# coralogix/arrow-ballista

Hardware: AMD Instinct MI355X
Metric: tpch_sf100_q3_lineitem_rows_per_sec (higher is better)
Workload: dtype i128; 1 GPU; TPC-H SF100 q3 (BASELINE configs[2]): filter x3 + hash join customer|x|orders + hash join |x| lineitem + aggregate + sort, one task on 1 x MI355X; lineitem_rows=600037902, lineitem_rows_per_gpu=600037902, orders_rows_per_gpu=150009476, customer_rows_per_gpu=15000000, input=Arrow-physical columns resident in HBM, parallelism=single partition

## Files before the change

### arrow-ballista_amd/csrc/agg_compile.cpp

```cpp
#include "agg_compile.h"
#include <algorithm>
#include <cctype>
#include <cstdio>
#include <functional>

namespace gpuq {

gpuq_field_info make_field(const std::string& name, const DType& t, bool nullable) {
  gpuq_field_info f{};
  std::snprintf(f.name, sizeof(f.name), "%s", name.c_str());
  f.type = t.id; f.precision = t.p; f.scale = t.s; f.nullable = nullable;
  f.repr = (t.id == T_UTF8) ? GPUQ_REPR_PACKED15 : GPUQ_REPR_ARROW;
  f.width = (t.id == T_BOOL) ? 0 : type_width(t);
  return f;
}

KeySpec make_keyspec(const std::vector<int>& regs, const std::vector<DType>& types, bool null_word) {
  if (regs.size() > (size_t)MAX_KEYS) throw Unsupported("more than " + std::to_string(MAX_KEYS) + " key columns");
  KeySpec K{};
  K.n_keys = (int)regs.size(); K.null_word = null_word ? 1 : 0;
  int w = 0;
  for (size_t k = 0; k < regs.size(); ++k) {
    K.key_reg[k] = regs[k];
    const bool wide = types[k].id == T_DECIMAL128 || types[k].id == T_UTF8;
// ... 395 lines not shown

}

AggCompiled compile_aggregate(const Schema& in, const Json& d) {
  AggCompiled R;
  R.mode = d.get_str("mode", "Single");
  const bool is_final = (R.mode == "Final" || R.mode == "FinalPartitioned");
  const bool emit_state = (R.mode == "Partial");
  if (!is_final && !emit_state && R.mode != "Single") throw std::runtime_error("unknown aggregate mode '" + R.mode + "'");
  R.strategy = d.get_str("strategy", "auto");
  R.expected_groups = d.get_i64("expected_groups", 0);
  Scan s(in);
  ExprCompiler& ec = s.ec;
  if (d.has("predicate")) ec.add_predicate(ec.from_json(d.at("predicate")));
  std::vector<NodeP> declared; std::vector<std::string> declared_names;
  if (d.has("group_expr")) for (const Json& g : d.at("group_expr").a) {
    declared.push_back(ec.from_json(g.at("expr"))); declared_names.push_back(g.get_str("name", "group" + std::to_string(declared.size() - 1)));
  }
  const GroupKeys keys(ec, declared, declared_names);
  R.refuse = keys.refuse;
  s.ungrouped = keys.nodes.empty();
  States states{ec, keys.declared(), in.fields.size()};
  std::vector<AggPlan> plans;
  for (const Json& a : d.at("aggr_expr").a) {
    s.fn = a.at("fn").str(); s.desc = &a;
    AggPlan pl; pl.name = a.get_str("name", s.fn);
    for (auto& ch : s.fn) ch = (char)std::toupper(ch);
    if (a.get_bool("distinct", false)) throw Unsupported("DISTINCT aggregates are not supported on device");
    pl.fn = find_agg_fn(s.fn);
    if (!is_final) {
      NodeP arg = a.has("expr") ? ec.from_json(a.at("expr")) : nullptr;
      if (a.has("filter") && !a.at("filter").is_null()) {
        NodeP p = ec.from_json(a.at("filter"));
        if (p->type.id != T_BOOL) throw std::runtime_error("aggregate FILTER must be boolean");
        if (!arg) arg = ec.lit_int(I64, 1);
        arg = ec.select(p, arg, ec.lit_null(arg->type));
        if (a.has("expr2")) throw Unsupported("FILTER on a two-argument aggregate");
      }
      if (!arg && !(pl.fn && pl.fn->args == 0)) throw std::runtime_error(s.fn + " needs an argument");
      if (!pl.fn) throw Unsupported("aggregate function " + s.fn);
      pl.fn->parts.from_args(s, pl, arg);
    } else {
      if (!pl.fn) throw Unsupported("aggregate function " + s.fn);
      pl.fn->parts.from_states(s, pl, states);
    }
    plans.push_back(pl);
  }
  std::vector<AccDef>& accs = s.accs;
  if (accs.empty()) s.count(nullptr);
  std::vector<int> key_slots, acc_slots(accs.size(), -1);
  for (auto& k : keys.nodes) key_slots.push_back(ec.add_output(k));
  for (size_t i = 0; i < accs.size(); ++i) if (accs[i].arg) acc_slots[i] = ec.add_output(accs[i].arg);
  R.prog = ec.finish();
  if (!s.origin_of.empty()) {
    if (d.has("predicate")) s.pick.add_predicate(ec.from_json(d.at("predicate")));
    R.pick = s.pick.finish();
    R.n_origins = (int)s.origin_of.size();
  }
  const int nk = (int)keys.nodes.size();
  R.agg.n_keys = nk; R.agg.n_accs = (int)accs.size();
  std::vector<int> kregs; bool any_null_key = false;
  for (int k = 0; k < nk; ++k) {
    const NodeP& n = keys.nodes[k];
    R.agg.key_reg[k] = R.prog.out_reg[key_slots[k]]; kregs.push_back(R.agg.key_reg[k]);
    R.key_types.push_back(n->type); any_null_key = any_null_key || n->nullable;
    if (n->type.id == T_BOOL || n->type.id == T_NULL) throw Unsupported("group-by key of type " + n->type.to_string());
  }
  for (size_t i = 0; i < accs.size(); ++i) {
    R.agg.acc_kind[i] = accs[i].kind; R.agg.acc_reg[i] = accs[i].arg ? R.prog.out_reg[acc_slots[i]] : 0;
    R.acc_types.push_back(accs[i].type);
    R.acc_bits.push_back(accs[i].arg ? R.prog.out_bits[acc_slots[i]] : 1);
  }
  R.keys = make_keyspec(kregs, R.key_types, any_null_key);
  {
    int total = 0; bool narrow = nk > 0;
    for (int k = 0; k < nk && narrow; ++k) {
      int bits = 0; bool sgn = false;
      switch (keys.nodes[k]->type.id) {
        case T_INT8: bits = 8; sgn = true; break;   case T_UINT8: bits = 8; break;
        case T_INT16: bits = 16; sgn = true; break; case T_UINT16: bits = 16; break;
        case T_INT32: case T_DATE32: bits = 32; sgn = true; break; case T_UINT32: bits = 32; break;
        default: narrow = false;
      }
      R.keys.sk_bits[k] = bits; R.keys.sk_signed[k] = sgn; R.keys.sk_null[k] = keys.nodes[k]->nullable ? 1 : 0;
      total += bits + R.keys.sk_null[k];
    }
    R.keys.state_key = narrow && total <= 62;
  }

  for (int k = 0; k < nk; ++k) { Field f; f.name = keys.names[k]; f.type = keys.nodes[k]->type; f.nullable = keys.nodes[k]->nullable; f.raw128 = 1; R.post_schema.fields.push_back(f); }
  for (size_t i = 0; i < accs.size(); ++i) { Field f; f.name = "acc" + std::to_string(i); f.type = accs[i].type; f.nullable = false; f.raw128 = 1; R.post_schema.fields.push_back(f); }
  std::function<void(size_t, size_t, bool)> emit = [&](size_t lo, size_t hi, bool with_keys) {
    ExprCompiler pc(R.post_schema);
    std::vector<std::string> names; CompiledProgram cp;
    try {
      if (with_keys) keys.project(pc, names);
      Post p{pc, nk, accs, names};
      for (size_t pi = lo; pi < hi; ++pi) (emit_state ? plans[pi].fn->parts.states : plans[pi].fn->parts.value)(p, plans[pi]);
      cp = pc.finish();
    }
    catch (const Unsupported&) { throw; }
    catch (const std::runtime_error&) {
      if (hi - lo + (with_keys ? 1 : 0) <= 1) throw;
      if (with_keys && hi > lo) { emit(lo, lo, true); emit(lo, hi, false); }
      else { const size_t mid = lo + (hi - lo) / 2; emit(lo, mid, with_keys); emit(mid, hi, false); }
      return;
// ... 12 lines not shown
```

### arrow-ballista_amd/csrc/agg_compile.h

```cpp
#pragma once
#include "../../include/gpuq.h"
#include "expr_compile.h"
#include "gpuq_kernels.h"
#include <string>
#include <vector>

namespace gpuq {

gpuq_field_info make_field(const std::string& name, const DType& t, bool nullable);
KeySpec make_keyspec(const std::vector<int>& regs, const std::vector<DType>& types, bool null_word);

struct AggCompiled {
  std::string mode = "Single", strategy = "auto";
  i64 expected_groups = 0;
  CompiledProgram prog;
  CompiledProgram pick; int n_origins = 0;
  AggSpec agg{}; KeySpec keys{};
  std::vector<DType> key_types, acc_types;
  std::vector<int> acc_bits;
  Schema post_schema;
  struct Post { CompiledProgram prog; int first_out = 0; };
  std::vector<Post> posts;
  std::vector<gpuq_field_info> out_fields;
  std::string refuse;
};
AggCompiled compile_aggregate(const Schema& in, const Json& descriptor);

}
```

### arrow-ballista_amd/csrc/capi.cpp

```cpp
#include "../../include/gpuq.h"
#include "expr_compile.h"
#include "agg_compile.h"
#include "gpuq_kernels.h"
#include "jit_runtime.h"
#include "devbuf.h"
#include "gpuq_internal.h"
#include <hip/hip_runtime.h>
#include <algorithm>
#include <memory>
#include <mutex>
#include <cctype>
#include <cstddef>
#include <cstdio>
#include <cstdlib>
#include <cstring>
#include <string>
#include <tuple>
#include <map>
#include <deque>
#include <functional>
#include <vector>

using namespace gpuq;

namespace {

thread_local std::string g_last_error;

u64 next_pow2(u64 v) { u64 r = 1; while (r < v) r <<= 1; return r; }

}


struct gpuq_timer { hipEvent_t a = nullptr, b = nullptr; };

enum OpKind { K_FILTER, K_PROJECT, K_AGG, K_JOIN_BUILD, K_JOIN_PROBE, K_SORT, K_PARTITION };

struct PassBufs {
  DevBuf hist, look; size_t look_bytes = 0;
  static size_t guess_word_at() { return (size_t)sort_max_passes() * 256; }
  u64* counts(bool with_guess_word = false) { return (u64*)hist.ensure((guess_word_at() + (with_guess_word ? 1 : 0)) * 8); }
  const u64* guess_word() const { return hist.as<u64>() + guess_word_at(); }
  void* lookback(i64 n) { look_bytes = onesweep_ws_bytes(n); return look.ensure(look_bytes); }
};

struct gpuq_op {
  gpuq_ctx* ctx = nullptr;
  OpKind kind = K_FILTER;
  Schema in_schema;
  CompiledProgram prog;
  DevBuf code_dev, flags_dev;
  std::vector<gpuq_field_info> out_fields;
  std::string mode = "Single", strategy = "auto";
  AggSpec agg{}; KeySpec keys{};
  std::vector<DType> key_types, acc_types;
  std::vector<int> acc_bits;
  std::map<std::pair<const void*, int>, int> jit_runs;
  std::map<std::tuple<const void*, int, size_t>, const JitFn*> jit_fns;
  struct PostChunk { CompiledProgram prog; DevBuf code; int first_out = 0; };
  std::deque<PostChunk> posts; Schema post_schema;
  CompiledProgram pick; DevBuf pick_code, origins_dev, origin_rows; int n_origins = 0;
  i64 expected_groups = 0;
  int agg_path = 0;
  int join_type = JT_INNER; int null_eq = 0; bool build_side_rows = true;
  bool has_semi = false; KeySpec semi_keys{};
  SortSpec sort{}; i64 fetch = -1;
  uint32_t nparts = 0;
  struct { void* data = nullptr; u64* valid = nullptr; bool done = false; } sort_dec;
  DType sort_key0;
  std::string refuse;
  std::string label;
  bool deferred = false, defer_client = false;
  struct Learned {
    struct { bool valid = false, dense = false, sparse_bits = false, has_dups = false; i64 kmin = 0; u64 krange = 0; } jb;
    struct { bool valid = false; int path = 0, gmax = 0; u64 est = 0; bool use_lds = false; i64 groups = -1; } ag;
    struct { bool valid = false; SortPack K{}; int total = 0; } so;
    bool join_guess_failed = false, sort_guess_failed = false;
    bool agg_runs_failed = false;
    uint32_t expect_flags = 0;
    void forget() { jb.valid = ag.valid = so.valid = false; }
  } learned;
  struct { DevBuf bitmap, counts, total; } w_filter;
  struct { DevBuf keys, key_nulls, cells, tiny, table, soa, sample, fstage, runs; } w_agg;
  struct { DevBuf key_range; } w_build;
  struct { DevBuf seg_build, seg_probe, counts, rec, rec2, hist, scan, locality; } w_probe;
  struct { DevBuf blocks, klo, klo2, khi, ids, ids2; PassBufs pass; DevBuf khi2, pairs; } w_sort;
  struct { DevBuf pid, pid2; PassBufs pass; DevBuf counts; } w_part;
  uint32_t* pin = nullptr;
  uint32_t* pinned() { if (!pin) { if (hipHostMalloc((void**)&pin, 256, hipHostMallocDefault) != hipSuccess) { (void)hipGetLastError(); pin = nullptr; } } return pin; }
  bool profile = false; hipEvent_t ev0 = nullptr, ev1 = nullptr; float kernel_ms = 0; int launches = 0; bool ev_pending = false;
  hipEvent_t ev2 = nullptr, ev3 = nullptr; float total_ms = 0, last_total_ms = 0; bool ev_total_pending = false;
  ~gpuq_op() { for (hipEvent_t e : {ev0, ev1, ev2, ev3}) if (e) (void)hipEventDestroy(e); if (pin) (void)hipHostFree(pin); }
};

struct gpuq_join_table {
  gpuq_ctx* ctx = nullptr;
  KeySpec keys{}; HashTable T{}; int null_eq = 0; bool has_present = true;
  DevBuf slots, dense, dense_bits, next, visited, present, ws_bitmap, ws_counts;
  i64 bound = 0;
  bool visited_ready = false;
  bool has_dups = false;
};

namespace {

template <class F> int guarded(gpuq_ctx*, F&& f) { return guarded_into(g_last_error, f); }

thread_local bool g_upload = true;
void upload_code(const CompiledProgram& p, DevBuf& dst) {
  if (!g_upload) return;
  dst.ensure(sizeof(DevCode));
  HIPCHECK(hipMemcpy(dst.p, &p.code, sizeof(DevCode), hipMemcpyHostToDevice));
}

DevProgram bind_program(const CompiledProgram& cp, const Schema& schema, const DevCode* code_dev, uint32_t* flags_dev, const gpuq_input* in) {
  if (!in) throw std::runtime_error("input is NULL");
  if (in->n_cols != (int)schema.fields.size())
    throw std::runtime_error("input has " + std::to_string(in->n_cols) + " columns, operator expects " + std::to_string(schema.fields.size()));
  if (in->n_via < 0 || in->n_via > MAX_VIA) throw std::runtime_error("n_via out of range");
  if (in->n_rows < 0 || in->n_rows > 0xFFFFFFFEll) throw std::runtime_error("n_rows out of range (max 2^32-2 positions per call)");
  DevProgram P{};
  P.n_cols = (int)cp.col_field.size(); P.n_insns = cp.n_insns; P.pred_reg = cp.pred_reg; P.n_via = in->n_via;
  for (int k = 0; k < in->n_via; ++k) { if (!in->via[k] && in->n_rows > 0) throw std::runtime_error("index vector is NULL"); P.via[k] = in->via[k]; }
  P.code = code_dev; P.flags = flags_dev; P.n_dev = (const u64*)in->n_rows_dev;
  for (size_t c = 0; c < cp.col_field.size(); ++c) {
    const int fi = cp.col_field[c];
    const Field& f = schema.fields[fi];
    const gpuq_column& col = in->cols[fi];
    if (col.type != f.type.id || (f.type.id == T_DECIMAL128 && (col.precision != f.type.p || col.scale != f.type.s)))
      throw std::runtime_error("column '" + f.name + "': type does not match the operator's input schema (" + f.type.to_string() + ")");
    if (f.side > in->n_via) throw std::runtime_error("column '" + f.name + "' needs index vector " + std::to_string(f.side));
    if (!col.data && col.length > 0 && in->n_rows > 0) throw std::runtime_error("column '" + f.name + "': data is NULL");
    if (!f.nullable && f.side == 0 && col.validity) {  }
    DevCol& d = P.cols[c];
    d.data = col.data; d.offsets = col.offsets; d.validity = col.validity;
    d.cls = f.raw128 ? CC_I128 : col_class_for(f.type);
    if (d.cls == CC_STR && !f.raw128 && !col.offsets && col.length > 0) throw std::runtime_error("Utf8 column '" + f.name + "' has no offsets");
    if (f.raw128 && f.type.id == T_UTF8) d.cls = CC_I128;
    if (d.cls == CC_STR && c < cp.col_loose.size() && cp.col_loose[c]) d.cls = CC_STRQ;
    d.via = f.side;
  }
  return P;
}

DevProgram bind_input(gpuq_op* op, const gpuq_input* in) { return bind_program(op->prog, op->in_schema, op->code_dev.as<DevCode>(), op->flags_dev.as<uint32_t>(), in); }
void check_payload_via(int payload_via, const gpuq_input* in) { if (payload_via < 0 || payload_via > in->n_via) throw std::runtime_error("payload_via out of range"); }
void check_row_limit(i64 n, const char* what) { if (n >= (1ll << 31)) throw Unsupported(std::string(what) + " of >= 2^31 rows in one call"); }
void need_exact_rows(const gpuq_input* in, const char* what) {
  if (in && in->n_rows_dev) throw std::runtime_error(std::string(what) + ": the input carries a device-side row count (n_rows_dev); this entry point needs the exact count");
}
struct OpStatus { uint32_t flags = 0, pad0 = 0, n_groups = 0, pad1 = 0; };
uint32_t* n_groups_dev(gpuq_op* op) { return op->flags_dev.as<uint32_t>() + offsetof(OpStatus, n_groups) / 4; }
void reset_flags(gpuq_op* op, hipStream_t s) { HIPCHECK(hipMemsetAsync(op->flags_dev.p, 0, 4, s)); }
OpStatus read_status(gpuq_op* op, hipStream_t s, int words = 4) {
  OpStatus st; uint32_t* h = op->pinned();
  HIPCHECK(hipMemcpyAsync(h ? (void*)h : (void*)&st, op->flags_dev.p, (size_t)words * 4, hipMemcpyDeviceToHost, s));
  HIPCHECK(hipStreamSynchronize(s));
  if (h) std::memcpy(&st, h, (size_t)words * 4);
  return st;
}
uint32_t read_flags(gpuq_op* op, hipStream_t s) { return read_status(op, s, 1).flags; }
void raise_flags(uint32_t f) {
  if (f & FLAG_STR_TRUNC) throw LongString("a Utf8 value longer than 15 bytes reached a device string comparison/key (PACKED15 limit)");
  if (f & FLAG_DEC_OVERFLOW) throw std::runtime_error("decimal arithmetic overflow: a result or a rescaled operand does not fit Decimal128 (38 digits / 127 bits)");
  if (f & FLAG_WIDE_MINMAX) throw Unsupported("MIN/MAX over a value outside the int64 range is not supported on device");
  if (f & FLAG_DUP_BUILD_KEY) throw Unsupported("duplicate build keys without a chain buffer");
  if (f & FLAG_OUT_OVERFLOW) throw Capacity("join output capacity exceeded; see the pair count for the required size");
  if (f & FLAG_TABLE_FULL) throw std::runtime_error("hash table full");
  if (f & FLAG_GROUP_OVERFLOW) throw Capacity("group capacity exceeded");
  if (f & FLAG_SORT_LAYOUT) throw std::runtime_error("a row does not fit the remembered sort key layout");
  if (f & FLAG_AGG_RUNS) throw std::runtime_error("the aggregate's input is not clustered on its key");
}
uint32_t raise_unless(gpuq_op* op, hipStream_t s, uint32_t f, uint32_t tolerated = 0) {
  if (f & ~tolerated) { reset_flags(op, s); raise_flags(f & ~tolerated); }
  return f & tolerated;
}

struct ProfScope {
  gpuq_op* op; hipStream_t s;
  ProfScope(gpuq_op* o, hipStream_t st) : op(o), s(st) {
    if (op->profile) {
      if (!op->ev0) { HIPCHECK(hipEventCreate(&op->ev0)); HIPCHECK(hipEventCreate(&op->ev1)); }
      if (op->ev_pending) { float ms = 0; HIPCHECK(hipEventSynchronize(op->ev1)); HIPCHECK(hipEventElapsedTime(&ms, op->ev0, op->ev1)); op->kernel_ms += ms; op->ev_pending = false; }
      HIPCHECK(hipEventRecord(op->ev0, s));
    }
  }
  ~ProfScope() { if (op->profile) { (void)hipEventRecord(op->ev1, s); op->ev_pending = true; op->launches++; } }
};

struct ProfTotal {
  gpuq_op* op; hipStream_t s; bool on = false;
  ProfTotal(gpuq_op* o, hipStream_t st) : op(o), s(st) {
    if (op->profile) {
      if (!op->ev2) { HIPCHECK(hipEventCreate(&op->ev2)); HIPCHECK(hipEventCreate(&op->ev3)); }
      if (op->ev_total_pending) {
        if (hipEventQuery(op->ev3) != hipSuccess) { (void)hipGetLastError(); return; }
        float ms = 0; HIPCHECK(hipEventElapsedTime(&ms, op->ev2, op->ev3)); op->total_ms += ms; op->ev_total_pending = false;
      }
// ... 28 lines not shown
    } catch (const std::exception& e) {
      if (c->jit_mode == 2) throw Unsupported(e.what());
      c->last_jit_error = e.what();
    }
  }
};

OutSpec make_outspec(const CompiledProgram& cp, gpuq_column* outs, int n_outs, const std::vector<gpuq_field_info>& fields) {
  if (n_outs != (int)cp.out_reg.size()) throw std::runtime_error("expected " + std::to_string(cp.out_reg.size()) + " output columns, got " + std::to_string(n_outs));
  if (n_outs > MAX_OUTS) throw Unsupported("more than " + std::to_string(MAX_OUTS) + " output columns in one call");
  OutSpec O{}; O.n_out = n_outs;
  for (int i = 0; i < n_outs; ++i) {
    if (!outs[i].data) throw std::runtime_error("output column " + std::to_string(i) + " has no data buffer");
    O.cols[i].data = const_cast<void*>(outs[i].data);
    O.cols[i].validity = (u64*)const_cast<uint8_t*>(outs[i].validity);
    O.cols[i].reg = cp.out_reg[i];
    O.cols[i].cls = col_class_for(cp.out_type[i]);
    outs[i].type = fields[i].type; outs[i].precision = fields[i].precision; outs[i].scale = fields[i].scale; outs[i].repr = fields[i].repr;
  }
  return O;
}

std::string agg_tiny_spec(const gpuq_op* op, int gmax) {
  const int nk = op->agg.n_keys, na = op->agg.n_accs;
  std::string spec = "#define GPUQ_JIT_SPEC 1\nconstexpr int JIT_NKEYS = " + std::to_string(nk) + ", JIT_NACCS = " + std::to_string(na) +
                     ", JIT_GMAX = " + std::to_string(gmax) + ", JIT_NKC = " + std::to_string(nk > 0 ? nk : 1) + ";\n";
  auto arr = [](const char* name, const int32_t* v, int n_) { std::string r = std::string("constexpr int ") + name + "[" + std::to_string(n_) + "] = {";
                                                             for (int i = 0; i < n_; ++i) r += std::to_string(v[i]) + (i + 1 < n_ ? "," : ""); return r + "};\n"; };
  int32_t bits[MAX_ACCS]; for (int i = 0; i < MAX_ACCS; ++i) bits[i] = i < (int)op->acc_bits.size() ? op->acc_bits[(size_t)i] : 127;
  return spec + arr("JIT_KEY_REG", op->agg.key_reg, MAX_KEYS) + arr("JIT_ACC_KIND", op->agg.acc_kind, MAX_ACCS) + arr("JIT_ACC_REG", op->agg.acc_reg, MAX_ACCS) +
         arr("JIT_ACC_BITS", bits, MAX_ACCS);
}

void check_ctx(gpuq_ctx* c) { if (!c) throw std::runtime_error("ctx is NULL"); HIPCHECK(hipSetDevice(c->device)); }

template <class F> int run_op(gpuq_op* op, OpKind kind, void* stream, F&& body) {
  static const char* const a_kind[] = {"a filter", "a project", "an aggregate", "a join_build", "a join_probe", "a sort", "a partition"};
  if (!op) return GPUQ_ERR_INVALID;
  return guarded(op->ctx, [&]() {
    check_ctx(op->ctx);
    if (op->kind != kind) throw std::runtime_error(std::string("not ") + a_kind[kind] + " operator");
    body(use_stream(stream));
  });
}

struct SelGeom { i64 nwords, wpb; int nblocks; };
SelGeom selection_geometry(const gpuq_ctx* ctx, i64 n) {
  const i64 nwords = (i64)words_of(n), maxb = (i64)ctx->cus * 8;
  const i64 wpb = std::max<i64>((nwords + maxb - 1) / maxb, 16);
  return {nwords, wpb, (int)((nwords + wpb - 1) / wpb)};
}

u64* bucket_records(hipStream_t s, u64* rec, u64* rec2, i64 n, int npass, const PassBufs& pass, uint32_t* ids_out, int last_mode) {
  for (int p = 0; p < npass; ++p) {
    const bool last = p + 1 == npass;
    launch_onesweep_pass(s, rec, nullptr, n, 32 + 8 * p, pass.hist.as<u64>() + (size_t)p * 256, pass.look.p, pass.look_bytes, rec2, last ? ids_out : nullptr, last ? last_mode : 0);
    std::swap(rec, rec2);
  }
  return rec;
}

}

extern "C" {

int gpuq_abi_version(void) { return GPUQ_ABI_VERSION; }

gpuq_ctx* gpuq_ctx_create(int device_ordinal, const char* json_opts) {
  gpuq_ctx* c = nullptr;
  int rc = guarded(nullptr, [&]() {
    int dev = device_ordinal;
    if (json_opts && *json_opts) { Json o = JsonParser(json_opts).parse(); dev = (int)o.get_i64("device", dev); }
    int count = 0;
    hipError_t e = hipGetDeviceCount(&count);
    if (e != hipSuccess || count <= 0) throw HipError("no usable HIP device (gpuq has no CPU fallback): " + std::string(hipGetErrorString(e)));
    if (dev < 0 || dev >= count) throw std::runtime_error("device ordinal out of range");
    HIPCHECK(hipSetDevice(dev));
    hipDeviceProp_t prop; HIPCHECK(hipGetDeviceProperties(&prop, dev));
    c = new gpuq_ctx();
    c->device = dev; c->cus = prop.multiProcessorCount; c->hbm = prop.totalGlobalMem; c->name = prop.name; c->arch = prop.gcnArchName;
    set_num_cus(c->cus);
    std::string jm = std::getenv("GPUQ_JIT") ? std::getenv("GPUQ_JIT") : "";
    if (json_opts && *json_opts) { Json o = JsonParser(json_opts).parse(); jm = o.get_str("jit", jm); c->jit_min_rows = o.get_i64("jit_min_rows", c->jit_min_rows); }
    if (jm == "off" || jm == "0") c->jit_mode = 0; else if (jm == "force" || jm == "2") c->jit_mode = 2; else c->jit_mode = 1;
    c->jit_wait = jm == "wait";
    if (!jit_available() && c->jit_mode == 1) c->jit_mode = 0;
    if (const char* e = std::getenv("GPUQ_JOIN_DENSE")) c->join_dense = std::atoi(e) != 0;
  });
  if (rc != GPUQ_OK) { delete c; return nullptr; }
  return c;
}
void gpuq_ctx_free(gpuq_ctx* ctx) { delete ctx; }
const char* gpuq_last_error(gpuq_ctx*) { return g_last_error.c_str(); }
int gpuq_last_refusal(void) { return tls_refusal(); }
int gpuq_ctx_device_info(gpuq_ctx* ctx, char* buf, size_t cap) {
  return guarded(ctx, [&]() {
    check_ctx(ctx);
    std::snprintf(buf, cap, "{\"name\":\"%s\",\"arch\":\"%s\",\"cus\":%d,\"hbm_bytes\":%zu}", ctx->name.c_str(), ctx->arch.c_str(), ctx->cus, ctx->hbm);
  });
}

static void compile_op(gpuq_op* op, const Json& d) {
    const std::string kind = d.at("op").str();
    for (char c : d.get_str("label", "")) if (std::isalnum((unsigned char)c) || c == '_') op->label += c;
    op->in_schema = schema_from_json(d.at("input"));
    if (kind == "filter") {
      op->kind = K_FILTER;
      ExprCompiler ec(op->in_schema); ec.add_predicate(ec.from_json(d.at("predicate")));
      op->prog = ec.finish(); upload_code(op->prog, op->code_dev);
    } else if (kind == "project") {
      op->kind = K_PROJECT;
      ExprCompiler ec(op->in_schema);
      std::vector<std::string> names;
      for (const Json& e : d.at("exprs").a) { ec.add_output(ec.from_json(e.at("expr"))); names.push_back(e.get_str("name", "col" + std::to_string(names.size()))); }
      op->prog = ec.finish(); upload_code(op->prog, op->code_dev);
      for (size_t i = 0; i < names.size(); ++i) op->out_fields.push_back(make_field(names[i], op->prog.out_type[i], op->prog.out_nullable[i]));
    } else if (kind == "aggregate") {
      op->kind = K_AGG;
      AggCompiled c = compile_aggregate(op->in_schema, d);
      op->mode = c.mode; op->strategy = c.strategy; op->expected_groups = c.expected_groups; op->refuse = c.refuse;
      op->prog = std::move(c.prog); upload_code(op->prog, op->code_dev);
      op->agg = c.agg; op->keys = c.keys;
      op->key_types = std::move(c.key_types); op->acc_types = std::move(c.acc_types); op->acc_bits = std::move(c.acc_bits);
      op->post_schema = std::move(c.post_schema); op->out_fields = std::move(c.out_fields);
      for (AggCompiled::Post& p : c.posts) {
        op->posts.emplace_back(); gpuq_op::PostChunk& pc = op->posts.back();
        pc.prog = std::move(p.prog); pc.first_out = p.first_out; upload_code(pc.prog, pc.code);
      }
      op->n_origins = c.n_origins;
      if (op->n_origins > 0) {
        op->pick = std::move(c.pick); upload_code(op->pick, op->pick_code);
        OriginPick O{}; O.n_origins = op->n_origins;
        for (int k = 0; k < op->n_origins; ++k) O.reg[k] = op->pick.out_reg[k];
        auto dsts_of = [&](const CompiledProgram& cp, DevBuf& code) {
          for (const auto& [k, slot] : cp.param_imm) {
            if (O.n_dsts >= MAX_ORIGIN_DSTS) throw Unsupported("aggregate reads its origins in more than " + std::to_string(MAX_ORIGIN_DSTS) + " places");
            O.dst_origin[O.n_dsts] = k; O.dst[O.n_dsts] = g_upload ? &code.as<DevCode>()->imm_lo[slot] : nullptr; ++O.n_dsts;
          }
        };
        dsts_of(op->prog, op->code_dev);
        for (auto& pc : op->posts) dsts_of(pc.prog, pc.code);
        if (g_upload) { op->origins_dev.ensure(sizeof(OriginPick)); HIPCHECK(hipMemcpy(op->origins_dev.p, &O, sizeof(OriginPick), hipMemcpyHostToDevice)); }
      }
    } else if (kind == "join_build" || kind == "join_probe") {
      op->kind = kind == "join_build" ? K_JOIN_BUILD : K_JOIN_PROBE;
      ExprCompiler ec(op->in_schema);
      if (d.has("predicate")) ec.add_predicate(ec.from_json(d.at("predicate")));
      std::vector<NodeP> ks;
      for (const Json& e : d.at("on").a) { NodeP n = ec.from_json(e); ks.push_back(n); ec.add_output(n); }
      if (ks.empty()) throw std::runtime_error("join needs at least one key");
      std::vector<NodeP> semi;
      if (d.has("semi_on")) {
        if (op->kind != K_JOIN_BUILD) throw std::runtime_error("semi_on belongs to a join_build operator");
        for (const Json& e : d.at("semi_on").a) { NodeP n = ec.from_json(e); semi.push_back(n); ec.add_output(n); }
      }
      op->prog = ec.finish(); upload_code(op->prog, op->code_dev);
      op->null_eq = d.get_bool("null_equals_null", false) ? 1 : 0;
      op->build_side_rows = d.get_bool("build_side_rows", true);
      std::vector<int> regs; for (size_t k = 0; k < ks.size(); ++k) { regs.push_back(op->prog.out_reg[k]); op->key_types.push_back(ks[k]->type); }
      op->keys = make_keyspec(regs, op->key_types, op->null_eq != 0);
      op->has_semi = !semi.empty();
      if (op->has_semi) {
        std::vector<int> sregs; std::vector<DType> stypes;
        for (size_t k = 0; k < semi.size(); ++k) { sregs.push_back(op->prog.out_reg[ks.size() + k]); stypes.push_back(semi[k]->type); }
        op->semi_keys = make_keyspec(sregs, stypes, op->null_eq != 0);
      }
      if (op->kind == K_JOIN_PROBE) {
        static const std::map<std::string, int> jt = {{"Inner", JT_INNER}, {"Left", JT_LEFT}, {"Right", JT_RIGHT}, {"Full", JT_FULL},
            {"LeftSemi", JT_LEFT_SEMI}, {"LeftAnti", JT_LEFT_ANTI}, {"RightSemi", JT_RIGHT_SEMI}, {"RightAnti", JT_RIGHT_ANTI}};
        auto it = jt.find(d.get_str("join_type", "Inner"));
        if (it == jt.end()) throw std::runtime_error("unknown join_type");
        op->join_type = it->second;
      }
    } else if (kind == "sort") {
// ... 61 lines not shown
  r += "],\"out_reg\":[";
  for (size_t i = 0; i < p.out_reg.size(); ++i) { if (i) r += ","; r += std::to_string(p.out_reg[i]); }
  r += "],\"out_type\":[";
  for (size_t i = 0; i < p.out_type.size(); ++i) { if (i) r += ","; r += "\"" + p.out_type[i].to_string() + "\""; }
  return r + "]}";
}

int gpuq_compile_check(const char* json, char* buf, size_t cap) {
  gpuq_op* op = nullptr;
  int rc = guarded(nullptr, [&]() {
    if (!json) throw std::runtime_error("json is NULL");
    Json d = JsonParser(json).parse();
    op = new gpuq_op();
    g_upload = false;
    compile_op(op, d);
    g_upload = true;
    std::string r = "{\"program\":" + describe_program(op->prog, op->in_schema);
    if (op->kind == K_AGG) {
      r += ",\"post\":" + describe_program(op->posts.front().prog, op->post_schema) + ",\"post_programs\":" + std::to_string(op->posts.size()) + ",\"posts\":[";
      for (size_t i = 0; i < op->posts.size(); ++i) { if (i) r += ","; r += describe_program(op->posts[i].prog, op->post_schema); }
      r += "],\"acc_kinds\":[";
      for (int a = 0; a < op->agg.n_accs; ++a) { if (a) r += ","; r += std::to_string(op->agg.acc_kind[a]); }
      r += std::string("],\"state_key\":") + (op->keys.state_key ? "true" : "false");
      if (op->n_origins > 0) {
        r += ",\"pick\":" + describe_program(op->pick, op->in_schema) + ",\"origin_imm\":[";
        for (size_t i = 0; i < op->prog.param_imm.size(); ++i) { if (i) r += ","; r += "[" + std::to_string(op->prog.param_imm[i].first) + "," + std::to_string(op->prog.param_imm[i].second) + "]"; }
        r += "]";
      }
    }
    r += ",\"outputs\":[";
    for (size_t i = 0; i < op->out_fields.size(); ++i) {
      const gpuq_field_info& f = op->out_fields[i];
      if (i) r += ",";
      DType t; t.id = f.type; t.p = f.precision; t.s = f.scale;
      r += std::string("{\"name\":\"") + f.name + "\",\"type\":\"" + t.to_string() + "\",\"nullable\":" + (f.nullable ? "true" : "false") + "}";
    }
    r += "]}";
    if (buf && cap) { std::snprintf(buf, cap, "%s", r.c_str()); if (r.size() + 1 > cap) throw Capacity("describe buffer too small"); }
  });
  g_upload = true;
  delete op;
  return rc;
}
int gpuq_compile_jit_source(const char* json, int kernel_id, char* buf, size_t cap) {
  gpuq_op* op = nullptr;
  int rc = guarded(nullptr, [&]() {
    if (!json) throw std::runtime_error("json is NULL");
    Json d = JsonParser(json).parse();
    op = new gpuq_op();
    g_upload = false;
    compile_op(op, d);
    g_upload = true;
    std::string eval = op->prog.jit_src;
    if (kernel_id == GPUQ_SINK_AGG_TINY && op->kind == K_AGG) eval += agg_tiny_spec(op, (int)d.get_i64("jit_gmax", 4));
    const std::string src = jit_full_source(eval, kernel_id);
    if (src.size() + 1 > cap) throw Capacity("source needs " + std::to_string(src.size() + 1) + " bytes");
    std::memcpy(buf, src.c_str(), src.size() + 1);
  });
  g_upload = true;
  delete op;
  return rc;
}
void gpuq_op_free(gpuq_op* op) { delete op; }
int gpuq_op_num_outputs(gpuq_op* op) { return op ? (int)op->out_fields.size() : 0; }
int gpuq_op_output_field(gpuq_op* op, int i, gpuq_field_info* out) {
  if (!op || !out || i < 0 || i >= (int)op->out_fields.size()) return GPUQ_ERR_INVALID;
  *out = op->out_fields[i]; return GPUQ_OK;
}
int gpuq_op_check(gpuq_op* op, void* stream) {
  if (!op) return GPUQ_ERR_INVALID;
  return guarded(op->ctx, [&]() { check_ctx(op->ctx); hipStream_t s = use_stream(stream); raise_unless(op, s, read_flags(op, s)); });
}
int gpuq_op_set_deferred(gpuq_op* op, int on) { if (!op) return GPUQ_ERR_INVALID; op->deferred = on != 0; op->defer_client = true; return GPUQ_OK; }
int gpuq_op_can_defer(gpuq_op* op) {
  if (!op) return 0;
  switch (op->kind) {
    case K_FILTER: case K_PROJECT: case K_JOIN_PROBE: return 1;
    case K_JOIN_BUILD: return op->learned.jb.valid ? 1 : 0;
    case K_AGG: return op->learned.ag.valid ? 1 : 0;
    case K_SORT: return op->learned.so.valid ? 1 : 0;
    default: return 0;
  }
}
int gpuq_ops_settle(gpuq_ctx* ctx, void* stream, gpuq_op* const* ops, int n_ops, const uint64_t* const* words, int n_words, uint64_t* words_out) {
  return guarded(ctx, [&]() {
    check_ctx(ctx);
    if (n_ops < 0 || n_words < 0 || (n_ops && !ops) || (n_words && (!words || !words_out))) throw std::runtime_error("settle: bad arguments");
    hipStream_t s = use_stream(stream);
    const int total = n_ops + n_words;
    struct Blocks { u64* host = nullptr; DevBuf dev; size_t cap = 0; };
    thread_local Blocks B;
    if ((size_t)total > B.cap) {
      if (B.host) (void)hipHostFree(B.host);
      B.cap = (size_t)std::max(total, 256); B.host = nullptr;
      HIPCHECK(hipHostMalloc((void**)&B.host, B.cap * 8, hipHostMallocDefault));
    }
    u64* dev = (u64*)B.dev.ensure(B.cap * 8);
    for (int base = 0; base < total; base += 64) {
      GatherWords g{}; g.n = std::min(64, total - base);
      for (int i = 0; i < g.n; ++i) { const int k = base + i; g.src[i] = k < n_ops ? (const u64*)ops[k]->flags_dev.p : (const u64*)words[k - n_ops]; if (!g.src[i]) throw std::runtime_error("settle: NULL word"); }
      launch_gather_words(s, g, dev + base);
    }
    HIPCHECK(hipGetLastError());
    if (total > 0) HIPCHECK(hipMemcpyAsync(B.host, dev, (size_t)total * 8, hipMemcpyDeviceToHost, s));
    HIPCHECK(hipStreamSynchronize(s));
    for (int i = 0; i < n_words; ++i) words_out[i] = B.host[n_ops + i];
// ... 122 lines not shown
        const int no = (int)pc.prog.out_reg.size();
        std::vector<gpuq_field_info> fi(op->out_fields.begin() + pc.first_out, op->out_fields.begin() + pc.first_out + no);
        OutSpec O = make_outspec(pc.prog, outs + pc.first_out, no, fi);
        { SinkJit jit(op, pc.prog, GPUQ_SINK_PROJECT, rows); launch_project(s, jit.fn, PP, rows, O); }
      }
    };
    auto launch_tiny = [&](const int gmax, const bool reset) {
      int nb = 0; const size_t wsb = agg_tiny_workspace_bytes(gmax, nk, na, &nb);
      void* wsp = op->w_agg.tiny.ensure(wsb);
      alloc_raw(64);
      if (reset) reset_flags(op, s);
      const std::string spec = agg_tiny_spec(op, gmax);
      { SinkJit jit(op, op->prog, GPUQ_SINK_AGG_TINY, n, spec); ProfScope ps(op, s); launch_agg_tiny(s, jit.fn, P, n, op->agg, gmax, wsp); }
      launch_agg_tiny_merge(s, P, n, op->agg, gmax, wsp, raw);
    };
    HashTable T{};
    T.key_words = op->keys.key_words; T.slot_words = 1 + T.key_words + 2 * na;
    auto launch_table = [&](const u64 est, const u64 slot_pct, const bool use_lds, const bool reset) {
      Krun.state_key = (op->keys.state_key && !use_lds) ? 1 : 0;
      Krun.key_words = Krun.state_key ? 0 : op->keys.key_words;
      T.key_words = Krun.state_key ? 0 : op->keys.key_words; T.slot_words = 1 + T.key_words + 2 * na;
      T.n_slots = next_pow2(est * slot_pct / 100);
      T.slots = (u64*)op->w_agg.table.ensure((size_t)T.n_slots * T.slot_words * 8);
      launch_ht_init(s, T, &op->agg);
      if (reset) reset_flags(op, s);
      if (use_lds) {
        int n_fsum = 0; for (int a = 0; a < na; ++a) n_fsum += op->agg.acc_kind[a] == ACC_FSUM;
        u64* fstage = nullptr;
        const size_t fbytes = (size_t)T.n_slots * (size_t)n_fsum * (size_t)agg_lds_grid(n) * 8;
        if (n_fsum > 0 && fbytes <= ((size_t)256 << 20)) { fstage = (u64*)op->w_agg.fstage.ensure(fbytes); HIPCHECK(hipMemsetAsync(fstage, 0, fbytes, s)); }
        SinkJit jit(op, op->prog, GPUQ_SINK_AGG_LDS, n); ProfScope ps(op, s); launch_agg_lds(s, jit.fn, P, n, op->keys, op->agg, T, fstage, n_fsum);
      }
      else { SinkJit jit(op, op->prog, GPUQ_SINK_AGG_HASH, n); ProfScope ps(op, s); launch_agg_hash(s, jit.fn, P, n, Krun, op->agg, T); }
    };
    auto extract = [&]() {
      const bool direct = Krun.state_key && raw.cap > 0;
      if (direct) { layout_soa((uint32_t)raw.cap, true); soa_filled = true; }
      launch_agg_hash_extract(s, Krun, op->agg, T, raw, op->flags_dev.as<uint32_t>(), direct ? &soa : nullptr);
    };
    bool runs_ok = nk > 0 && op->keys.state_key;
    for (int a = 0; a < na; ++a) {
      const int kd = op->agg.acc_kind[a];
      runs_ok = runs_ok && (kd == ACC_SUM || kd == ACC_COUNT || kd == ACC_COUNT_STAR || kd == ACC_BAND || kd == ACC_BOR || kd == ACC_BXOR);
    }
    RunsGeom G{};
    auto launch_runs_count = [&](const bool reset) {
      Krun = op->keys;
      G = agg_runs_geometry(n);
      const size_t segs = (size_t)std::max<int32_t>(G.nsegs, 1);
      G.seg_last = (u64*)op->w_agg.runs.ensure(segs * 20 + 16); G.seg_first = G.seg_last + segs; G.counts = (uint32_t*)(G.seg_first + segs);
      raw.n_groups = n_groups_dev(op);
      if (reset) reset_flags(op, s);
      if (G.nsegs <= 0) { HIPCHECK(hipMemsetAsync(raw.n_groups, 0, 8, s)); return; }
      { SinkJit jit(op, op->prog, GPUQ_SINK_AGG_RUNS_COUNT, n); launch_agg_runs_count(s, jit.fn, P, n, Krun, G); }
      launch_scan_block_counts(s, G.counts, G.nsegs, (u64*)raw.n_groups);
      launch_agg_runs_order(s, G, op->flags_dev.as<uint32_t>());
    };
    auto launch_runs_write = [&](const i64 rcap) {
      raw.cap = (int32_t)rcap;
      layout_soa((uint32_t)rcap, true); soa_filled = true;
      if (na > 0) HIPCHECK(hipMemsetAsync(soa.acc_col[0], 0, (size_t)na * (size_t)rcap * 16, s));
      for (int a = 0; a < na; ++a) if (op->agg.acc_kind[a] == ACC_BAND) launch_fill_cells(s, soa.acc_col[a], rcap, ~0ull, 0);
      SinkJit jit(op, op->prog, GPUQ_SINK_AGG_RUNS_WRITE, n); ProfScope ps(op, s);
      launch_agg_runs_write(s, jit.fn, P, n, Krun, op->agg, G, soa, (uint32_t)rcap);
    };
    auto run_radix = [&](const std::string& strat, const i64 known_groups) -> bool {
      const int slot_words = 1 + op->keys.key_words + 2 * na;
      uint32_t capslots = 64; while ((size_t)capslots * 2 * slot_words * 8 <= 60 * 1024) capslots *= 2;
      if ((size_t)capslots * slot_words * 8 <= 60 * 1024 && n < (1ll << 31)) {
        const u64 est = op->expected_groups > 0 ? (u64)op->expected_groups : (known_groups > 0 ? (u64)known_groups + (u64)known_groups / 4 : (u64)n);
        const u64 per_bucket = std::max<u64>(1, (u64)capslots / 2);
        u64 nbk = next_pow2(std::max<u64>(1, (est + per_bucket - 1) / per_bucket)); if (nbk > (1ull << 24)) nbk = 1ull << 24;
        if (n >= (1ll << 20) && nbk < 2048) nbk = 2048;
        int bits = 0; while ((1ull << bits) < nbk) ++bits;
        DevBuf b_bid, b_bid2, b_ids; PassBufs pass; DevBuf b_bounds;
        u64* bid = (u64*)b_bid.ensure((size_t)n * 8); u64* bid2 = (u64*)b_bid2.ensure((size_t)n * 8);
        uint32_t* ids = (uint32_t*)b_ids.ensure((size_t)n * 4 + 16);
        u64* ghist = pass.counts();
        pass.lookback(n);
        uint32_t* bounds = (uint32_t*)b_bounds.ensure((size_t)(nbk + 2) * 4);
        reset_flags(op, s);
        { SinkJit jit(op, op->prog, GPUQ_SINK_AGG_BUCKET_ID, n); launch_agg_bucket_id(s, jit.fn, P, n, op->keys, nbk - 1, bid, nullptr); }
        const int npass = std::max(1, (bits + 7) / 8);
        launch_radix_ghist(s, bid, n, 32, npass, ghist);
        bid = bucket_records(s, bid, bid2, n, npass, pass, ids, 2);
        launch_bucket_bounds(s, bid, n, nbk, bounds, 32);
        alloc_raw((i64)std::min<u64>((u64)std::max<i64>(n, 1), std::max<u64>(est + est / 4, 1ull << 20)));
        { SinkJit jit(op, op->prog, GPUQ_SINK_AGG_BUCKET, n); ProfScope ps(op, s); launch_agg_bucket(s, jit.fn, P, op->keys, op->agg, ids, bounds, (uint32_t)nbk, capslots, slot_words, raw); }
        HIPCHECK(hipGetLastError());
        const OpStatus st = read_status(op, s);
        if (!raise_unless(op, s, st.flags, FLAG_TABLE_FULL | FLAG_GROUP_OVERFLOW)) { ng = st.n_groups; return true; }
        if (strat == "radix" && op->expected_groups > 0 && est < (u64)n) throw Capacity("radix aggregate: a bucket overflowed; raise expected_groups or use strategy hash/auto");
        reset_flags(op, s);
      } else if (strat == "radix") throw Unsupported("radix aggregate: the group state does not fit an LDS table");
      return false;
    };
    auto finish_on_device = [&]() {
      run_post((uint32_t)raw.cap, raw.n_groups);
      HIPCHECK(hipGetLastError());
      for (int i = 0; i < n_outs; ++i) outs[i].length = raw.cap;
      if (n_groups_out) *n_groups_out = raw.cap;
      *ndev_out = (const uint64_t*)raw.n_groups;
    };
    auto& L = op->learned;
    if (ndev_out && op->deferred && L.ag.valid) {
      if (L.ag.path == 1) {
        if (cap >= 64) { launch_tiny(L.ag.gmax, false); op->agg_path = 1; finish_on_device(); return; }
      } else if (L.ag.path == 2) {
        const u64 est = std::min<u64>(std::max<u64>(L.ag.est, 64), (u64)(L.ag.groups + L.ag.groups / 4 + 64));
// ... 495 lines not shown
      SortPack K = op->learned.so.K; K.check = 2;
      sort_with_plan(op, s, P, n, K, op->learned.so.total, perm_out);
      return;
    }
    if (in->n_rows_dev) throw std::runtime_error("sort: a device-side row count needs a deferred operator with a completed synchronous run (gpuq_op_can_defer)");
    op->learned.so.valid = false;
    static const bool spec_on = []() { const char* e = getenv("GPUQ_SORT_SPECULATE"); return !(e && e[0] == '0'); }();
    bool spec = spec_on && n >= (1ll << 22) && !op->learned.sort_guess_failed;
    for (int k = 0; k < S.n_keys; ++k) if (S.kind[k] == 2) spec = false;
    if (spec) {
      const i64 wstep = std::max<i64>(1, (i64)words_of(n) >> 12);
      const SortPack G = sort_key_plan(op, s, P, n, &total, wstep);
      if (total > 0) {
        sort_with_plan(op, s, P, n, G, total, perm_out);
        u64 failed = 0; uint32_t eflags = 0;
        HIPCHECK(hipMemcpyAsync(&failed, op->w_sort.pass.guess_word(), 8, hipMemcpyDeviceToHost, s));
        HIPCHECK(hipMemcpyAsync(&eflags, op->flags_dev.p, 4, hipMemcpyDeviceToHost, s));
        HIPCHECK(hipStreamSynchronize(s));
        raise_unless(op, s, eflags);
        if (!failed) { op->learned.so = {true, G, total}; op->learned.expect_flags = 0; return; }
        op->learned.sort_guess_failed = true;
      }
    }
    const SortPack K = sort_key_plan(op, s, P, n, &total);
    sort_with_plan(op, s, P, n, K, total, perm_out);
    op->learned.so = {true, K, total}; op->learned.expect_flags = 0;
  });
}

static void sort_with_plan(gpuq_op* op, hipStream_t s, const DevProgram& P, const i64 n, const SortPack& K_in, const int total, uint32_t* perm_out) {
  {
    SortPack K = K_in; K.total_bits = total;
    const SortSpec& S = op->sort;
    const bool packed = total >= 1 && total <= 32 && n > sort_small_max();
    auto& W = op->w_sort;
    u64* klo = (u64*)W.klo.ensure((size_t)n * 8);
    u64* klo2 = (u64*)W.klo2.ensure((size_t)n * 8);
    u64* khi = total > 64 ? (u64*)W.khi.ensure((size_t)n * 8) : nullptr;
    uint32_t* ids = packed ? nullptr : (uint32_t*)W.ids.ensure((size_t)n * 4);
    uint32_t* ids2 = packed ? nullptr : (uint32_t*)W.ids2.ensure((size_t)n * 4);
    ProfScope ps(op, s);
    const int np_all = (total + 7) / 8;
    u64* ghist = W.pass.counts(true);
    const bool small = n <= sort_small_max();
    const int dec_width = (op->sort_dec.data && S.n_keys == 1 && S.kind[0] == 0 && K.rshift[0] == 0 && total >= 1 && total <= 64 && !small) ? type_width(op->sort_key0) : 0;
    const bool decode = dec_width == 1 || dec_width == 2 || dec_width == 4 || dec_width == 8 || (dec_width == 16 && op->sort_key0.id == T_DECIMAL128);
    { SinkJit jit(op, op->prog, GPUQ_SINK_SORT_PACK, n); launch_sort_pack(s, jit.fn, P, n, S, K, klo, khi, ids, small || total == 0 ? nullptr : ghist, np_all); }
    if (small) {
      launch_sort_small(s, klo, khi, ids, n, perm_out);
      HIPCHECK(hipGetLastError());
      return;
    }
    void* lws = W.pass.lookback(n); const size_t lwb = W.pass.look_bytes;
    auto run_passes = [&](int bits, int shift0, int pass0, bool last_word) {
      const int np = (bits + 7) / 8;
      if (np == 0) { if (last_word) HIPCHECK(hipMemcpyAsync(perm_out, ids, (size_t)n * 4, hipMemcpyDeviceToDevice, s)); return; }
      for (int p = 0; p < np; ++p) {
        const bool final_pass = last_word && p + 1 == np;
        launch_onesweep_pass(s, klo, ids, n, shift0 + 8 * p, ghist + (size_t)(pass0 + p) * 256, lws, lwb, klo2, final_pass ? perm_out : ids2, final_pass ? (decode ? (packed ? 2 : 0) : 1) : 0);
        std::swap(klo, klo2); if (!final_pass) std::swap(ids, ids2);
      }
    };
    if (packed) {
      run_passes(total, 32, 0, true);
      if (decode) { launch_sort_decode(s, klo, 32, n, K, S.desc[0], S.nulls_first[0], dec_width, op->sort_dec.data, op->sort_dec.valid); op->sort_dec.done = true; }
    } else if (decode) {
      run_passes(total, 0, 0, true);
      launch_sort_decode(s, klo, 0, n, K, S.desc[0], S.nulls_first[0], dec_width, op->sort_dec.data, op->sort_dec.valid); op->sort_dec.done = true;
    } else {
      run_passes(std::min(total, 64), 0, 0, total <= 64);
      if (total > 64) {
        launch_gather_u64(s, khi, ids, n, klo);
        run_passes(total - 64, 0, 8, true);
      }
    }
    HIPCHECK(hipGetLastError());
  }
}

int gpuq_merge_run(gpuq_op* op, void* stream, const gpuq_input* in, const int64_t* run_offsets, int n_runs, uint32_t* perm_out) {
  return run_op(op, K_SORT, stream, [&](hipStream_t s) {
    if (!run_offsets || n_runs < 1) throw std::runtime_error("run_offsets is NULL / no runs");
    need_exact_rows(in, "merge");
    const i64 n = in->n_rows;
    if (run_offsets[0] != 0 || run_offsets[n_runs] != n) throw std::runtime_error("run_offsets must start at 0 and end at the row count");
    for (int r = 0; r < n_runs; ++r) if (run_offsets[r] > run_offsets[r + 1]) throw std::runtime_error("run_offsets must not decrease");
    if (n == 0) return;
    check_row_limit(n, "merge");
    if (!perm_out) throw std::runtime_error("perm_out is NULL");
    DevProgram P = bind_input(op, in);
    int total = 0;
    const SortPack K = sort_key_plan(op, s, P, n, &total);
    {
      int live = 0; for (int r = 0; r < n_runs; ++r) live += run_offsets[r + 1] > run_offsets[r];
      int rounds = 0; while ((1 << rounds) < live) ++rounds;
      const double est_merge = rounds * (total > 64 ? 1.9 : 1.45);
      const double est_passes = ((total + 7) / 8) * (total <= 32 ? 0.65 : 1.0) + (total > 64 ? 1.0 : 0.0);
      static const bool force_rounds = []() { const char* e = std::getenv("GPUQ_MERGE_ROUNDS"); return e && std::string(e) == "force"; }();
      if (live > 1 && est_passes < est_merge && !force_rounds) { sort_with_plan(op, s, P, n, K, total, perm_out); return; }
    }
    auto& W = op->w_sort;
    u64* klo = (u64*)W.klo.ensure((size_t)n * 8);
    u64* klo2 = (u64*)W.klo2.ensure((size_t)n * 8);
    u64* khi = total > 64 ? (u64*)W.khi.ensure((size_t)n * 8) : nullptr;
    u64* khi2 = total > 64 ? (u64*)W.khi2.ensure((size_t)n * 8) : nullptr;
    uint32_t* ids = (uint32_t*)W.ids.ensure((size_t)n * 4);
    uint32_t* ids2 = (uint32_t*)W.ids2.ensure((size_t)n * 4);
    ProfScope ps(op, s);
    { SinkJit jit(op, op->prog, GPUQ_SINK_SORT_PACK, n); launch_sort_pack(s, jit.fn, P, n, op->sort, K, klo, khi, ids, nullptr, 0); }
    std::vector<i64> bounds; bounds.push_back(0);
    for (int r = 0; r < n_runs; ++r) if (run_offsets[r + 1] > run_offsets[r]) bounds.push_back(run_offsets[r + 1]);
    i64* dpairs = (i64*)W.pairs.ensure((size_t)(bounds.size() + 2) * 3 * 8);
    while (bounds.size() > 2) {
      std::vector<i64> pairs, next; next.push_back(0); i64 max_len = 0;
// ... 738 lines not shown
```

### arrow-ballista_amd/csrc/expr_compile.cpp

```cpp
#include "expr_compile.h"
#include "devbuf.h"
#include <algorithm>
#include <cctype>
#include <cmath>
#include <functional>
#include <set>

namespace gpuq {

i128 pow10_i128(int k) { i128 r = 1; for (int i = 0; i < k; ++i) r *= 10; return r; }
int bits_for_precision(int p) { int b = (int)std::ceil(p * 3.3219280948873626) + 1; return b > 127 ? 127 : b; }
static int bits_of_value(i128 v) {
  u128 m = v < 0 ? (u128)(-(v + 1)) + 1 : (u128)v;
  int b = 0; while (m) { ++b; m >>= 1; }
  return b + 1 > 127 ? 127 : b + 1;
}
i128 parse_i128(const std::string& s) {
  size_t i = 0; bool neg = false;
  while (i < s.size() && s[i] == ' ') ++i;
  if (i < s.size() && (s[i] == '-' || s[i] == '+')) { neg = s[i] == '-'; ++i; }
  i128 v = 0; bool any = false;
  for (; i < s.size(); ++i) {
    if (s[i] < '0' || s[i] > '9') throw std::runtime_error("bad integer literal '" + s + "'");
    v = v * 10 + (s[i] - '0'); any = true;
// ... 676 lines not shown
      }
    };
    if (pred_) { if (pred_->kind == Node::LIT && pred_->lit_long) throw std::runtime_error(msg); chk(pred_.get()); }
    for (auto& o : outs_) { if (o->kind == Node::LIT && o->lit_long) throw std::runtime_error(msg); chk(o.get()); }
  }
  if (pred_) topo(pred_.get());
  for (auto& o : outs_) topo(o.get());
  for (Node* n : order) if (n->kind == Node::COL) {
    if ((int)C.col_field.size() >= MAX_COLS) throw std::runtime_error("expression references more than " + std::to_string(MAX_COLS) + " columns");
    reg[n] = (int)C.col_field.size();
    C.col_field.push_back(n->col);
  }
  C.col_loose.assign(C.col_field.size(), false);
  for (size_t c = 0; c < C.col_field.size(); ++c) {
    const Field& f = schema_.fields[C.col_field[c]];
    if (f.type.id != T_UTF8 || f.raw128) continue;
    bool loose = true;
    auto is_this = [&](Node* m) { return m->kind == Node::COL && m->col == C.col_field[c]; };
    if (pred_ && is_this(rep(pred_.get()))) loose = false;
    for (auto& o : outs_) if (is_this(rep(o.get()))) loose = false;
    for (Node* n : order) {
      if (n->kind != Node::OPN) continue;
      for (size_t k = 0; k < n->ch.size(); ++k) {
        if (!is_this(rep(n->ch[k].get()))) continue;
        if (n->op == OP_ISNULL || n->op == OP_ISNOTNULL) continue;
        const bool eq_lit = (n->op == OP_EQ || n->op == OP_NE) && n->ch.size() == 2 && rep(n->ch[1 - k].get())->kind == Node::LIT;
        const bool prefix_substr = n->op == OP_SUBSTR && ((n->imm >> 8) & 0xFFu) != 255u && (n->imm & 0xFFu) + ((n->imm >> 8) & 0xFFu) <= 15u;
        if (!eq_lit && !prefix_substr) loose = false;
      }
    }
    C.col_loose[c] = loose;
  }
  std::vector<bool> busy(NREG, false);
  for (size_t i = 0; i < C.col_field.size(); ++i) busy[i] = true;
  auto alloc = [&]() { for (int r = 0; r < NREG; ++r) if (!busy[r]) { busy[r] = true; return r; } throw std::runtime_error("expression needs more than " + std::to_string(NREG) + " live registers"); return -1; };
  std::vector<std::pair<u64, u64>> imms;
  std::vector<bool> imm_is_param;
  auto imm_new = [&](u64 lo, u64 hi, bool is_param) {
    if ((int)imms.size() >= MAX_IMMS) throw std::runtime_error("expression needs more than " + std::to_string(MAX_IMMS) + " immediates");
    imms.push_back({lo, hi}); imm_is_param.push_back(is_param); return (int)imms.size() - 1;
  };
  auto imm_index = [&](u64 lo, u64 hi) {
    for (size_t i = 0; i < imms.size(); ++i) if (!imm_is_param[i] && imms[i].first == lo && imms[i].second == hi) return (int)i;
    return imm_new(lo, hi, false);
  };
  param_slot_.clear();
  auto emit = [&](int op, int d, int a, int b, uint32_t imm) {
    if (C.n_insns >= MAX_INSNS) throw std::runtime_error("expression program longer than " + std::to_string(MAX_INSNS) + " instructions");
    DevInsn& in = C.code.insns[C.n_insns++];
    in.op = (uint8_t)op; in.dst = (uint8_t)d; in.a = (uint8_t)a; in.b = (uint8_t)b; in.imm = imm;
  };
  std::map<Node*, int> remaining = uses;
  auto release = [&](Node* c0) { Node* c = rep(c0); if (--remaining[c] == 0) busy[reg[c]] = false; };
  for (Node* n : order) {
    if (n->kind == Node::COL) continue;
    if (n->kind == Node::LIT) {
      const int d = alloc(); reg[n] = d;
      if (n->param >= 0) { const int slot = imm_new(0, 0, true); param_slot_[n] = slot; C.param_imm.push_back({n->param, slot}); emit(OP_IMM, d, 0, 0, (uint32_t)slot); continue; }
      if (n->lit_null) { emit(OP_IMM, d, 0, 0, (uint32_t)imm_index(0, 0)); emit(OP_NULLIF0, d, d, d, 0); }
      else emit(OP_IMM, d, 0, 0, (uint32_t)imm_index(n->lit_lo, n->lit_hi));
      continue;
    }
    const int a = n->ch.size() > 0 ? reg.at(rep(n->ch[0].get())) : 0;
    const int b = n->ch.size() > 1 ? reg.at(rep(n->ch[1].get())) : a;
    uint32_t imm = n->imm;
    if (n->op == OP_SELECT) imm = (uint32_t)reg.at(rep(n->ch[2].get()));
    for (auto& c : n->ch) release(c.get());
    const int d = alloc(); reg[n] = d;
    emit(n->op, d, a, b, imm);
  }
  for (size_t i = 0; i < imms.size(); ++i) { C.code.imm_lo[i] = imms[i].first; C.code.imm_hi[i] = imms[i].second; }
  C.pred_reg = pred_ ? reg.at(rep(pred_.get())) : -1;
  for (auto& o : outs_) {
    C.out_reg.push_back(reg.at(rep(o.get()))); C.out_type.push_back(o->type); C.out_nullable.push_back(o->nullable); C.out_key.push_back(o->key); C.out_bits.push_back((o->type.is_int() || o->type.is_decimal() || o->type.id == T_DATE32) ? o->bits : 127);
  }
  for (Node* n : order) if (n->kind == Node::OPN && (n->op == OP_ADDC || n->op == OP_SUBC || n->op == OP_MULC)) C.checks_overflow = true;
  C.jit_src = jit_source(C, order, reg);
  return C;
}

std::string ExprCompiler::jit_source(const CompiledProgram& C, const std::vector<Node*>& order, const std::map<Node*, int>& ) {
  auto rep = [](Node* n) { while (n->kind == Node::OPN && n->op == OP_MOV) n = n->ch[0].get(); return n; };
  std::string S;
  auto L = [&](const std::string& l) { S += "  " + l + "\n"; };
  std::map<Node*, std::string> name;
  std::map<Node*, std::string> nul;
  auto is_str = [](const Node* n) { return n->type.id == T_UTF8; };
  auto is_f = [](const Node* n) { return n->type.is_float(); };
  auto is_b = [](const Node* n) { return n->type.id == T_BOOL; };
  auto wide = [&](const Node* n) { return !is_str(n) && !is_f(n) && !is_b(n) && n->bits > 64; };
  auto ctype = [&](const Node* n) { return is_f(n) ? std::string("double") : (is_b(n) ? std::string("bool") : (wide(n) ? std::string("i128") : std::string("i64"))); };
  std::string SP, SLD, FP, FR;
  auto LP = [&](const std::string& l) { SP += "  " + l + "\n"; };
  auto LL = [&](const std::string& l) { SLD += "  " + l + "\n"; };
  auto fieldP = [&](const std::string& ty, const std::string& nm) { FP += "  " + ty + " " + nm + ";\n"; };
  std::string touch;
  auto fieldR = [&](const std::string& ty, const std::string& nm) {
    FR += "  " + ty + " " + nm + ";\n";
    if (ty == "ulonglong2") touch += "  asm volatile(\"\" :: \"v\"(w." + nm + ".x), \"v\"(w." + nm + ".y));\n";
    else if (ty != "bool") touch += "  asm volatile(\"\" :: \"v\"(w." + nm + "));\n";
  };
  bool via_used[MAX_VIA + 1] = {false, false, false, false};
  for (size_t c = 0; c < C.col_field.size(); ++c) via_used[schema_.fields[C.col_field[c]].side] = true;
  LP("const uint32_t row0 = (uint32_t)pos; (void)row0;");
  LL("const uint32_t row0 = (uint32_t)pos; (void)row0;");
  L("const uint32_t row0 = (uint32_t)pos; (void)row0;");
  for (int k = 1; k <= MAX_VIA; ++k) if (via_used[k]) {
    const std::string ks = std::to_string(k);
    fieldP("uint32_t", "row" + ks);
    LP("q.row" + ks + " = P.via[" + std::to_string(k - 1) + "][pos];");
    LL("const uint32_t row" + ks + " = q.row" + ks + ";");
  }
  std::vector<bool> narrow128(C.col_field.size(), false);
  for (size_t c = 0; c < C.col_field.size(); ++c) {
    const Field& f = schema_.fields[C.col_field[c]];
    const int cls = f.raw128 ? (int)CC_I128 : col_class_for(f.type);
    if (cls != CC_I128 || f.type.id == T_UTF8) continue;
    bool all_narrow = true, seen = false;
    for (Node* n : order) if (n->kind == Node::COL && n->col == C.col_field[c]) { seen = true; if (wide(n)) all_narrow = false; }
    narrow128[c] = seen && all_narrow;
  }
  for (size_t c = 0; c < C.col_field.size(); ++c) {
    const Field& f = schema_.fields[C.col_field[c]];
    const std::string cs = std::to_string(c), row = "row" + std::to_string(f.side);
    LL("const DevCol& col" + cs + " = P.cols[" + cs + "];");
    L("const DevCol& col" + cs + " = P.cols[" + cs + "]; (void)col" + cs + ";");
    if (f.side > 0) {
      LL("const bool ok" + cs + " = " + row + " != NULL_ROW;"); LL("const uint32_t r" + cs + " = ok" + cs + " ? " + row + " : 0u;");
      fieldR("bool", "ok" + cs); LL("w.ok" + cs + " = ok" + cs + ";"); L("const bool ok" + cs + " = w.ok" + cs + ";");
      fieldR("uint32_t", "r" + cs); LL("w.r" + cs + " = r" + cs + ";"); L("const uint32_t r" + cs + " = w.r" + cs + "; (void)r" + cs + ";");
    } else { LL("const uint32_t r" + cs + " = row0;"); L("const uint32_t r" + cs + " = row0; (void)r" + cs + ";"); }
    if (f.nullable) {
      LL("w.vb" + cs + " = (col" + cs + ".validity ? col" + cs + ".validity : (const uint8_t*)P.code)[col" + cs + ".validity ? (r" + cs + " >> 3) : 0u];");
      fieldR("uint32_t", "vb" + cs); L("const uint32_t vb" + cs + " = w.vb" + cs + ";");
    }
    const int cls = f.raw128 ? (int)CC_I128 : col_class_for(f.type);
    const std::string A = "a" + cs;
    switch (cls) {
      case CC_I32: case CC_U32: fieldR("uint32_t", A); LL("w." + A + " = " + std::string(f.side == 0 ? "GPUQ_LD_STREAM" : "*") + "(((const uint32_t*)col" + cs + ".data) + r" + cs + ");"); L("const uint32_t " + A + " = w." + A + ";"); break;
      case CC_I64: fieldR("u64", A); LL("w." + A + " = " + std::string(f.side == 0 ? "GPUQ_LD_STREAM" : "*") + "(((const u64*)col" + cs + ".data) + r" + cs + ");"); L("const u64 " + A + " = w." + A + ";"); break;
      case CC_I128:
        if (narrow128[c]) {
          fieldR("u64", A); LL("w." + A + " = ((const u64*)col" + cs + ".data)[2 * (size_t)r" + cs + "];"); L("const ulonglong2 " + A + " = make_ulonglong2(w." + A + ", 0ull);");
        } else { fieldR("ulonglong2", A); LL("w." + A + " = ((const ulonglong2*)col" + cs + ".data)[r" + cs + "];"); L("const ulonglong2 " + A + " = w." + A + ";"); }
        break;
      case CC_BIT: fieldR("uint32_t", A); LL("w." + A + " = ((const uint8_t*)col" + cs + ".data)[r" + cs + " >> 3];"); L("const uint32_t " + A + " = w." + A + ";"); break;
      case CC_F32: fieldR("uint32_t", A); LL("w." + A + " = " + std::string(f.side == 0 ? "GPUQ_LD_STREAM" : "*") + "(((const uint32_t*)col" + cs + ".data) + r" + cs + ");"); L("const uint32_t " + A + " = w." + A + ";"); break;
      case CC_I8: case CC_U8: fieldR("uint32_t", A); LL("w." + A + " = ((const uint8_t*)col" + cs + ".data)[r" + cs + "];"); L("const uint32_t " + A + " = w." + A + ";"); break;
      case CC_I16: case CC_U16: fieldR("uint32_t", A); LL("w." + A + " = ((const uint16_t*)col" + cs + ".data)[r" + cs + "];"); L("const uint32_t " + A + " = w." + A + ";"); break;
      case CC_STR: {
        const std::string oa = "o" + cs + "a", ob = "o" + cs + "b";
        fieldR("int32_t", oa); fieldR("int32_t", ob);
        if (f.side == 0) {
          fieldP("int32_t", oa); fieldP("int32_t", ob);
          LP("q." + oa + " = P.cols[" + cs + "].offsets[row0]; q." + ob + " = P.cols[" + cs + "].offsets[row0 + 1];");
          LL("w." + oa + " = q." + oa + "; w." + ob + " = q." + ob + ";");
          fieldR("u64", "sw" + cs + "a"); fieldR("u64", "sw" + cs + "b"); fieldR("u64", "sw" + cs + "c");
          LL("{ const unsigned long long sa = (unsigned long long)col" + cs + ".data + (unsigned long long)(uint32_t)q." + oa + "; const int sl = q." + ob + " - q." + oa + "; const uint32_t sn = (uint32_t)(sl < 15 ? sl : 15), span = (uint32_t)(sa & 7ull) + sn;");
          LL("  const u64* swp = (const u64*)(sa & ~7ull); const u64* dummy = (const u64*)P.code;");
          LL("  w.sw" + cs + "a = *(sl > 0 ? swp : dummy); w.sw" + cs + "b = *(span > 8u ? swp + 1 : dummy); w.sw" + cs + "c = *(span > 16u ? swp + 2 : dummy); }");
        } else {
          LL("w." + oa + " = col" + cs + ".offsets[r" + cs + "]; w." + ob + " = col" + cs + ".offsets[r" + cs + " + 1];");
        }
        L("const int32_t " + oa + " = w." + oa + ", " + ob + " = w." + ob + ";");
        break;
      }
    }
  }
  for (size_t c = 0; c < C.col_field.size(); ++c) {
    const Field& f = schema_.fields[C.col_field[c]];
    if (f.raw128 || f.type.id != T_UTF8) continue;
    const std::string cs = std::to_string(c);
    L("const int32_t len" + cs + " = o" + cs + "b - o" + cs + "a;");
    L("const uint8_t* sp" + cs + " = (const uint8_t*)col" + cs + ".data + o" + cs + "a;");
    (void)0;
  }
  std::map<int, std::string> col_null;
  for (Node* n : order) {
    if (n->kind != Node::COL) continue;
    int c = -1; for (size_t k = 0; k < C.col_field.size(); ++k) if (C.col_field[k] == n->col) c = (int)k;
    const Field& f = schema_.fields[n->col];
    const std::string cs = std::to_string(c);
    std::string nn = "false";
    if (f.nullable || (f.side > 0 && !f.dense)) {
      std::string e;
      if (f.side > 0 && !f.dense) e = "!ok" + cs;
      if (f.nullable) e += std::string(e.empty() ? "" : " || ") + "(col" + cs + ".validity && !((vb" + cs + " >> (r" + cs + " & 7)) & 1u))";
      L("const bool n_c" + cs + " = " + e + ";");
      nn = "n_c" + cs;
    }
    nul[n] = nn;
    const int cls = f.raw128 ? (int)CC_I128 : col_class_for(f.type);
    if (is_str(n)) {
      if (f.raw128) { L("const u64 c" + cs + "_lo = a" + cs + ".x, c" + cs + "_hi = a" + cs + ".y;"); }
      else {
        if (!(c < C.col_loose.size() && C.col_loose[c])) L("if (len" + cs + " > 15 && P.flags) atomicOr(P.flags, FLAG_STR_TRUNC);");
        L("u64 c" + cs + "_hi, c" + cs + "_lo;");
        if (f.side == 0) L("str15_assemble(w.sw" + cs + "a, w.sw" + cs + "b, w.sw" + cs + "c, (uint32_t)(((unsigned long long)col" + cs + ".data + (unsigned long long)(uint32_t)o" + cs + "a) & 7ull), len" + cs + " < 15 ? len" + cs + " : 15, c" + cs + "_hi, c" + cs + "_lo);");
        else L("load_str15((const uint8_t*)col" + cs + ".data, o" + cs + "a, len" + cs + ", c" + cs + "_hi, c" + cs + "_lo);");
        L("c" + cs + "_lo |= (u64)(len" + cs + " < 255 ? len" + cs + " : 255);");
      }
      name[n] = "c" + cs;
      continue;
    }
    std::string v;
    switch (cls) {
      case CC_I32: v = "(i64)(int32_t)a" + cs; break;
      case CC_U32: case CC_U8: case CC_U16: v = "(i64)a" + cs; break;
      case CC_I8: v = "(i64)(int8_t)a" + cs; break;
      case CC_I16: v = "(i64)(int16_t)a" + cs; break;
      case CC_F32: v = "(double)__uint_as_float(a" + cs + ")"; break;
      case CC_I64: v = is_f(n) ? "__longlong_as_double((i64)a" + cs + ")" : "(i64)a" + cs; break;
      case CC_I128:
        if (is_f(n)) v = "__longlong_as_double((i64)a" + cs + ".x)";
        else if (is_b(n)) v = "(a" + cs + ".x != 0)";
        else v = wide(n) ? "mk128(a" + cs + ".x, a" + cs + ".y)" : "(i64)a" + cs + ".x";
        break;
      case CC_BIT: v = "(((a" + cs + " >> (r" + cs + " & 7)) & 1u) != 0)"; break;
    }
    L("const " + ctype(n) + " c" + cs + " = " + v + ";");
    name[n] = "c" + cs;
  }
  int vid = 0;
  auto V = [&](const NodeP& x) {
// ... 90 lines not shown
      case OP_NOT: e = "!" + V(a); ne = N(a); break;
      case OP_ISNULL: e = "(" + N(a) + ")"; ne = "false"; break;
      case OP_ISNOTNULL: e = "!(" + N(a) + ")"; ne = "false"; break;
      case OP_SELECT: {
        const NodeP& f = n->ch[2];
        L("const bool " + t + "_c = !(" + N(a) + ") && " + V(a) + ";");
        if (is_str(n)) { L("const u64 " + t + "_lo = " + t + "_c ? " + V(b) + "_lo : " + V(f) + "_lo, " + t + "_hi = " + t + "_c ? " + V(b) + "_hi : " + V(f) + "_hi;"); two_vars = true; }
        else e = "(" + t + "_c ? (" + T + ")" + V(b) + " : (" + T + ")" + V(f) + ")";
        ne = (N(b) == "false" && N(f) == "false") ? "false" : "(" + t + "_c ? (" + N(b) + ") : (" + N(f) + "))";
        break;
      }
      case OP_SHL: e = "(i128)((u128)" + as128(a) + " << " + std::to_string(n->imm) + ")"; ne = N(a); break;
      case OP_DATEPART: e = "date_part_of_days((i64)" + V(a) + ", " + std::to_string(n->imm) + ")"; ne = N(a); break;
      case OP_SUBSTR: {
        L("bool " + t + "_bad = false; const u128 " + t + "_x = substr_packed(((u128)" + V(a) + "_hi << 64) | (u128)" + V(a) + "_lo, " + std::to_string(n->imm & 0xFFu) + "u, " +
          std::to_string((n->imm >> 8) & 0xFFu) + "u, " + t + "_bad);");
        L("if (" + t + "_bad && !(" + N(a) + ") && P.flags) atomicOr(P.flags, FLAG_STR_TRUNC);");
        L("const u64 " + t + "_lo = (u64)" + t + "_x, " + t + "_hi = (u64)(" + t + "_x >> 64);");
        two_vars = true; ne = N(a); break;
      }
      case OP_BOR: e = "(" + as128(a) + " | " + as128(b) + ")"; break;
      case OP_BAND: e = "(" + as128(a) + " & " + as128(b) + ")"; break;
      case OP_BXOR: e = "(" + as128(a) + " ^ " + as128(b) + ")"; break;
      case OP_FFLOOR: e = "floor(" + V(a) + ")"; ne = N(a); break;
      case OP_FCEIL: e = "ceil(" + V(a) + ")"; ne = N(a); break;
      case OP_FTRUNC: e = "trunc(" + V(a) + ")"; ne = N(a); break;
      case OP_WRAP: e = "wrap_int((i128)" + V(a) + ", " + std::to_string(n->imm) + "u)"; ne = N(a); break;
      case OP_ADDC: case OP_SUBC: case OP_MULC: {
        L("bool " + t + "_o; const i128 " + t + "_v = checked_arith(" + std::to_string(n->op) + ", " + as128(a) + ", " + as128(b) + ", " + ((n->imm & 1u) ? "true" : "false") + ", " + t + "_o);");
        L("if (" + t + "_o && !(" + ne + ") && P.flags) atomicOr(P.flags, FLAG_DEC_OVERFLOW);");
        e = t + "_v"; break;
      }
      case OP_NULLIF0: {
        Node* rb = rep(b.get());
        const std::string bz = is_str(rb) ? "(" + V(b) + "_lo == 0 && " + V(b) + "_hi == 0)" : (is_f(rb) ? "(__double_as_longlong(" + V(b) + ") == 0)" : "(" + V(b) + " == 0)");
        if (is_str(n)) { L("const u64 " + t + "_lo = " + V(a) + "_lo, " + t + "_hi = " + V(a) + "_hi;"); two_vars = true; } else e = "(" + T + ")" + V(a);
        ne = orn({N(a), N(b), bz}); break;
      }
      case OP_COALESCE0:
        if (is_str(n)) { L("const u64 " + t + "_lo = (" + N(a) + ") ? 0 : " + V(a) + "_lo, " + t + "_hi = (" + N(a) + ") ? 0 : " + V(a) + "_hi;"); two_vars = true; }
        else e = "((" + N(a) + ") ? (" + T + ")0 : (" + T + ")" + V(a) + ")";
        ne = "false"; break;
      default: throw std::runtime_error("jit: unsupported op " + std::to_string(n->op));
    }
    if (!two_vars) L("const " + T + " " + t + " = (" + T + ")" + e + ";");
    if (!n->nullable || ne == "false") nul[n] = "false";
    else { L("const bool " + t + "_n = " + ne + ";"); nul[n] = t + "_n"; }
    name[n] = t;
    emit_pred();
  }
  emit_pred();
  L("uint32_t nm = 0;");
  std::set<int> done;
  for (size_t k = 0; k < outs_.size(); ++k) {
    Node* o = rep(outs_[k].get());
    const int r = C.out_reg[k];
    if (done.count(r)) continue;
    done.insert(r);
    const std::string rs = std::to_string(r);
    if (is_str(o)) L("rlo[" + rs + "] = " + name.at(o) + "_lo; rhi[" + rs + "] = " + name.at(o) + "_hi;");
    else if (is_f(o)) L("rlo[" + rs + "] = (u64)__double_as_longlong(" + name.at(o) + "); rhi[" + rs + "] = 0;");
    else if (is_b(o)) L("rlo[" + rs + "] = " + name.at(o) + " ? 1ull : 0ull; rhi[" + rs + "] = 0;");
    else if (wide(o)) L("rlo[" + rs + "] = (u64)" + name.at(o) + "; rhi[" + rs + "] = (u64)((u128)" + name.at(o) + " >> 64);");
    else L("rlo[" + rs + "] = (u64)" + name.at(o) + "; rhi[" + rs + "] = (u64)(" + name.at(o) + " >> 63);");
    if (nul.at(o) != "false") L("if (" + nul.at(o) + ") nm |= " + std::to_string(1u << r) + "u;");
  }
  L("rnulls = nm;");
  L("return true;");
  std::string R = "struct JitPre {\n" + FP + "  int32_t pad_;\n};\nstruct JitRaw {\n" + FR + "  int32_t pad_;\n};\n";
  R += "__device__ __forceinline__ void gpuq_jit_pre(const DevProgram& P, i64 pos, JitPre& q) {\n" + SP + "  (void)P; (void)q;\n}\n";
  R += "__device__ __forceinline__ void gpuq_jit_load(const DevProgram& P, i64 pos, const JitPre& q, JitRaw& w) {\n" + SLD + "  (void)q; (void)w;\n}\n";
  R += "__device__ __forceinline__ bool gpuq_jit_compute(const DevProgram& P, i64 pos, const JitRaw& w, GPUQ_REGS_PARAM) {\n" + touch + S + "}\n";
  R += "__device__ __forceinline__ bool gpuq_jit_eval(const DevProgram& P, i64 pos, GPUQ_REGS_PARAM) {\n"
       "  JitPre q; gpuq_jit_pre(P, pos, q);\n  JitRaw w; gpuq_jit_load(P, pos, q, w);\n  return gpuq_jit_compute(P, pos, w, GPUQ_REGS);\n}\n";
  return R;
}

}
```

### arrow-ballista_amd/csrc/expr_compile.h

```cpp
#pragma once
#include "gpuq_dev.h"
#include "json.h"
#include <map>
#include <memory>
#include <string>
#include <vector>

namespace gpuq {

enum TypeId : int32_t {
  T_NULL = 0, T_BOOL = 1, T_INT32 = 2, T_INT64 = 3, T_DATE32 = 4, T_FLOAT64 = 5,
  T_DECIMAL128 = 6, T_UTF8 = 7, T_UINT32 = 8, T_UINT64 = 9,
  T_INT8 = 10, T_INT16 = 11, T_UINT8 = 12, T_UINT16 = 13, T_FLOAT32 = 14,
  T_TIMESTAMP = 15,
  T_DATE64 = 16,
};

struct DType {
  int32_t id = T_NULL;
  int32_t p = 0, s = 0;
  bool operator==(const DType& o) const { return id == o.id && (id != T_DECIMAL128 || (p == o.p && s == o.s)) && (id != T_TIMESTAMP || p == o.p); }
  bool operator!=(const DType& o) const { return !(*this == o); }
  bool is_int() const { return id == T_INT32 || id == T_INT64 || id == T_UINT32 || id == T_UINT64 || id == T_INT8 || id == T_INT16 || id == T_UINT8 || id == T_UINT16; }
  bool is_unsigned() const { return id == T_UINT8 || id == T_UINT16 || id == T_UINT32 || id == T_UINT64; }
  bool is_temporal() const { return id == T_DATE32 || id == T_DATE64 || id == T_TIMESTAMP; }
  bool is_decimal() const { return id == T_DECIMAL128; }
  bool is_float() const { return id == T_FLOAT64 || id == T_FLOAT32; }
  std::string to_string() const;
};
DType dtype_from_json(const Json& j);
Json dtype_to_json_text(const DType& t);
DType dtype_from_arrow_format(const char* f, bool* large_utf8);
std::string arrow_format_of(const DType& t);
int col_class_for(const DType& t);
int type_width(const DType& t);

struct Field {
  std::string name;
  DType type;
  bool nullable = true;
  int side = 0;
  int raw128 = 0;
  int dense = 0;
};
struct Schema {
  std::vector<Field> fields;
  int index_of(const std::string& name) const;
};
Schema schema_from_json(const Json& j);

struct Node;
typedef std::shared_ptr<Node> NodeP;
struct Node {
  enum Kind { COL, LIT, OPN } kind = LIT;
  int op = OP_NOP;
  std::vector<NodeP> ch;
  uint32_t imm = 0;
  DType type;
  bool nullable = true;
  int bits = 127;
  int col = -1;
  u64 lit_lo = 0, lit_hi = 0; bool lit_null = false;
  bool lit_long = false;
  int param = -1;
  std::string key;
};

struct CompiledProgram {
  DevCode code{};
  int n_insns = 0;
  std::vector<int> col_field;
  std::vector<bool> col_loose;
  int pred_reg = -1;
  std::vector<int> out_reg;
  std::vector<DType> out_type;
  std::vector<bool> out_nullable;
  std::vector<std::string> out_key;
  std::vector<int> out_bits;
  bool checks_overflow = false;
  std::vector<std::pair<int, int>> param_imm;
  std::string jit_src;
};

class ExprCompiler {
 public:
  explicit ExprCompiler(const Schema& schema) : schema_(schema) {}
  NodeP from_json(const Json& e);
  NodeP column(int field_index);
  NodeP lit_int(DType t, i128 v);
  NodeP lit_f64(double v);
  NodeP lit_f32(float v);
  NodeP param_f64(int k);
  NodeP floor_div(NodeP e, i64 d, DType rt);
  NodeP rescale_time(NodeP e, i64 from_per_s, i64 to_per_s, DType rt);
  NodeP lit_null(DType t);
  NodeP lit_str(const std::string& s);
  NodeP binary(const std::string& op, NodeP l, NodeP r);
  NodeP cast(NodeP e, DType to);
  NodeP not_(NodeP e);
  NodeP is_null(NodeP e, bool negate);
  NodeP negative(NodeP e);
  NodeP select(NodeP c, NodeP t, NodeP f);
  NodeP raw(int op, DType t, bool nullable, int bits, std::vector<NodeP> ch, uint32_t imm = 0);
  NodeP rescale(NodeP e, int new_scale);
  NodeP wrap_to(NodeP e, DType t, int bits, bool may_be_negative);
  NodeP coalesce0(NodeP e);
  NodeP nullif0(NodeP e, NodeP guard);
  void add_predicate(NodeP e);
  int add_output(NodeP e);
  CompiledProgram finish();
  const Schema& schema() const { return schema_; }

 private:
  Schema schema_;
  NodeP pred_;
  std::vector<NodeP> outs_;
  std::map<std::string, NodeP> interned_;
  std::map<const Node*, int> param_slot_;
  NodeP intern(NodeP n);
  std::string jit_source(const CompiledProgram& C, const std::vector<Node*>& order, const std::map<Node*, int>& reg);
};

i128 pow10_i128(int k);
int bits_for_precision(int p);
i128 parse_i128(const std::string& s);
std::string i128_to_string(i128 v);
bool pack_str15(const std::string& s, u64& lo, u64& hi);

}
```

### arrow-ballista_amd/csrc/gpuq_dev.h

```cpp
#pragma once
#ifndef __HIPCC_RTC__
#include <hip/hip_runtime.h>
#include <stdint.h>
#else
typedef signed char int8_t;
typedef unsigned char uint8_t;
typedef signed short int16_t;
typedef unsigned short uint16_t;
typedef signed int int32_t;
typedef unsigned int uint32_t;
#endif

namespace gpuq {

typedef unsigned long long u64;
typedef long long i64;
typedef __int128 i128;
typedef unsigned __int128 u128;

constexpr int MAX_COLS = 16;
constexpr int NREG = 16;
constexpr int MAX_INSNS = 192;
constexpr int MAX_IMMS = 48;
constexpr int MAX_VIA = 3;
constexpr uint32_t NULL_ROW = 0xFFFFFFFFu;

enum ColClass : int32_t {
  CC_I32 = 0,
  CC_I64 = 1,
  CC_I128 = 2,
  CC_STR = 3,
  CC_BIT = 4,
  CC_U32 = 5,
  CC_I8 = 7, CC_I16 = 8, CC_U8 = 9, CC_U16 = 10,
  CC_F32 = 11,
  CC_STRQ = 6,
};

struct DevCol {
  const void* data;
  const int32_t* offsets;
  const uint8_t* validity;
  int32_t cls;
  int32_t via;
};

enum Op : uint8_t {
  OP_NOP = 0,
  OP_IMM,
  OP_MOV,
  OP_ADD, OP_SUB, OP_MUL, OP_MULW , OP_NEG, OP_DIV , OP_MOD,
  OP_EQ, OP_NE, OP_LT, OP_LE, OP_GT, OP_GE,
  OP_FADD, OP_FSUB, OP_FMUL, OP_FDIV, OP_FNEG, OP_FSQRT,
  OP_FEQ, OP_FNE, OP_FLT, OP_FLE, OP_FGT, OP_FGE,
  OP_I2F, OP_F2I,
  OP_AND, OP_OR, OP_NOT,
  OP_ISNULL, OP_ISNOTNULL,
  OP_SELECT,
  OP_SHL,
  OP_BOR,
  OP_NULLIF0,
  OP_COALESCE0,
  OP_DATEPART,
  OP_SUBSTR,
  OP_F32R,
  OP_WRAP,
  OP_ADDC, OP_SUBC, OP_MULC,
  OP_BAND,
  OP_BXOR,
  OP_FFLOOR, OP_FCEIL, OP_FTRUNC,
};

struct DevInsn { uint8_t op, dst, a, b; uint32_t imm; };

struct DevCode {
  DevInsn insns[MAX_INSNS];
  u64 imm_lo[MAX_IMMS];
  u64 imm_hi[MAX_IMMS];
};

struct DevProgram {
  int32_t n_cols;
  int32_t n_insns;
  int32_t pred_reg;
  int32_t n_via;
  DevCol cols[MAX_COLS];
  const uint32_t* via[MAX_VIA];
  const DevCode* code;
  uint32_t* flags;
// ... 442 lines not shown
```

### arrow-ballista_amd/csrc/gpuq_kernels.h

```cpp
#pragma once
#include "gpuq_dev.h"
#ifndef GPUQ_JIT
#include <type_traits>
#include "devbuf.h"
#endif

namespace gpuq {

constexpr int MAX_OUTS = 16;
struct OutCol {
  void* data;
  u64* validity;
  int32_t reg;
  int32_t cls;
};
struct OutSpec { int32_t n_out; int32_t pad; OutCol cols[MAX_OUTS]; };

constexpr int MAX_ACCS = 12;
constexpr int MAX_KEYS = 4;
enum AccKind : int32_t { ACC_SUM = 0, ACC_COUNT = 1, ACC_COUNT_STAR = 2, ACC_MIN = 3, ACC_MAX = 4, ACC_FSUM = 5, ACC_FMIN = 6, ACC_FMAX = 7,
                         ACC_BAND = 8, ACC_BOR = 9, ACC_BXOR = 10  };
struct AggSpec {
  int32_t n_keys, n_accs;
  int32_t key_reg[MAX_KEYS];
// ... 231 lines not shown
#define GPUQ_SINK_JOIN_KEYRANGE 14
#define GPUQ_SINK_RJ_PACK 15
#define GPUQ_SINK_AGG_RUNS_COUNT 16
#define GPUQ_SINK_AGG_RUNS_WRITE 17

#ifndef GPUQ_JIT
struct SinkInfo { int id; const char* file; const char* entry; };
constexpr SinkInfo GPUQ_SINKS[] = {
    {GPUQ_SINK_FILTER_BITMAP, "kernels_scan.hip", "gpuq_jit_filter_bitmap"},
    {GPUQ_SINK_PROJECT, "kernels_scan.hip", "gpuq_jit_project"},
    {GPUQ_SINK_AGG_TINY, "kernels_scan.hip", "gpuq_jit_agg_tiny"},
    {GPUQ_SINK_AGG_HASH, "kernels_hash.hip", "gpuq_jit_agg_hash"},
    {GPUQ_SINK_JOIN_BUILD, "kernels_hash.hip", "gpuq_jit_join_build"},
    {GPUQ_SINK_JOIN_PROBE, "kernels_hash.hip", "gpuq_jit_join_probe"},
    {GPUQ_SINK_JOIN_PROBE_UNIQUE, "kernels_hash.hip", "gpuq_jit_join_probe_unique"},
    {GPUQ_SINK_SORT_MINMAX, "kernels_sort.hip", "gpuq_jit_sort_minmax"},
    {GPUQ_SINK_SORT_PACK, "kernels_sort.hip", "gpuq_jit_sort_pack"},
    {GPUQ_SINK_PART_PID, "kernels_sort.hip", "gpuq_jit_part_pid"},
    {GPUQ_SINK_AGG_BUCKET_ID, "kernels_hash.hip", "gpuq_jit_agg_bucket_id"},
    {GPUQ_SINK_AGG_BUCKET, "kernels_hash.hip", "gpuq_jit_agg_bucket"},
    {GPUQ_SINK_AGG_LDS, "kernels_hash.hip", "gpuq_jit_agg_lds"},
    {GPUQ_SINK_JOIN_KEYRANGE, "kernels_hash.hip", "gpuq_jit_join_keyrange"},
    {GPUQ_SINK_RJ_PACK, "kernels_hash.hip", "gpuq_jit_rj_pack"},
    {GPUQ_SINK_AGG_RUNS_COUNT, "kernels_hash.hip", "gpuq_jit_agg_runs_count"},
    {GPUQ_SINK_AGG_RUNS_WRITE, "kernels_hash.hip", "gpuq_jit_agg_runs_write"},
};
void launch_gather_words(hipStream_t s, const GatherWords& g, u64* out);
void set_num_cus(int n);
int num_cus();
int grid_for_words(i64 n, int waves_per_block, int blocks_per_cu);
void launch_filter_bitmap(hipStream_t s, void* jit_fn, const DevProgram& P, i64 n, u64* bitmap, uint32_t* block_counts, int nblocks, i64 words_per_block);
void launch_scan_block_counts(hipStream_t s, uint32_t* block_counts, int nblocks, u64* total_out);
void launch_compact(hipStream_t s, const u64* bitmap, const uint32_t* block_offsets, int nblocks, i64 words_per_block, i64 n,
                    const uint32_t* sel_in, uint32_t* sel_out);
void launch_project(hipStream_t s, void* jit_fn, const DevProgram& P, i64 n, const OutSpec& O);
int agg_tiny_max_groups(int n_accs);
size_t agg_tiny_workspace_bytes(int gmax, int n_keys, int n_accs, int* nblocks_out);
void launch_agg_tiny(hipStream_t s, void* jit_fn, const DevProgram& P, i64 n, const AggSpec& A, int gmax, void* workspace);
void launch_agg_tiny_merge(hipStream_t s, const DevProgram& P, i64 n, const AggSpec& A, int gmax, void* workspace, const AggOut& out);
void launch_ht_init(hipStream_t s, const HashTable& T, const AggSpec* A);
void launch_agg_hash(hipStream_t s, void* jit_fn, const DevProgram& P, i64 n, const KeySpec& K, const AggSpec& A, const HashTable& T);
void launch_key_sample(hipStream_t s, const DevProgram& P, i64 n, const KeySpec& K, i64 stride, i64 nsample, uint32_t* bitmap, u64 nbits, unsigned long long* passed);
void launch_agg_origin_pick(hipStream_t s, const DevProgram& pick, i64 n, const OriginPick* origins_dev, unsigned int* first_row);
uint32_t agg_lds_slots(const HashTable& T);
int agg_lds_grid(i64 n);
void launch_agg_lds(hipStream_t s, void* jit_fn, const DevProgram& P, i64 n, const KeySpec& K, const AggSpec& A, const HashTable& T, u64* fstage, int n_fsum);
void launch_agg_bucket_id(hipStream_t s, void* jit_fn, const DevProgram& P, i64 n, const KeySpec& K, u64 bucket_mask, u64* bid, uint32_t* ids);
void launch_bucket_bounds(hipStream_t s, const u64* sorted_bid, i64 n, u64 nbuckets, uint32_t* bounds, int shift);
void launch_agg_bucket(hipStream_t s, void* jit_fn, const DevProgram& P, const KeySpec& K, const AggSpec& A, const uint32_t* ids, const uint32_t* bounds, uint32_t nbuckets,
                       uint32_t cap, int slot_words, const AggOut& out);
void launch_agg_hash_extract(hipStream_t s, const KeySpec& K, const AggSpec& A, const HashTable& T, const AggOut& out, uint32_t* flags, const AggSoA* soa = nullptr);
RunsGeom agg_runs_geometry(i64 n);
void launch_agg_runs_count(hipStream_t s, void* jit_fn, const DevProgram& P, i64 n, const KeySpec& K, const RunsGeom& G);
void launch_agg_runs_order(hipStream_t s, const RunsGeom& G, uint32_t* flags);
void launch_agg_runs_write(hipStream_t s, void* jit_fn, const DevProgram& P, i64 n, const KeySpec& K, const AggSpec& A, const RunsGeom& G, const AggSoA& soa, uint32_t cap);
void launch_fill_cells(hipStream_t s, ulonglong2* cells, i64 n, u64 lo, u64 hi);
bool launch_join_build(hipStream_t s, void* jit_fn, const DevProgram& P, i64 n, const KeySpec& K, const HashTable& T, uint32_t* next, uint32_t* present,
                       int payload_via, int null_equals_null, const SemiProbe* semi = nullptr);
void launch_join_keyrange(hipStream_t s, void* jit_fn, const DevProgram& P, i64 n, const KeySpec& K, int null_equals_null, u64* out, i64 wstep = 1);
void launch_join_probe_unique(hipStream_t s, void* jit_fn, const DevProgram& P, i64 n, const KeySpec& K, const HashTable& T, int join_type, int null_equals_null, int payload_via,
                              uint32_t* seg_build, uint32_t* seg_probe, uint32_t* seg_counts, int nsegs, i64 wpw, uint32_t* visited);
void launch_copy_segments(hipStream_t s, const uint32_t* seg_build, const uint32_t* seg_probe, const uint32_t* seg_offsets, int nsegs, i64 wpw, i64 n,
                          const u64* total, uint32_t* out_build, uint32_t* out_probe, u64 out_cap, uint32_t* flags);
void launch_join_locality(hipStream_t s, const DevProgram& P, i64 n, const KeySpec& K, const HashTable& T, i64 stride, i64 nsample, u64* out);
struct RjGeomHost { uint32_t nparts, shift; i64 tile; int32_t nblocks; };
void rj_geometry(i64 n, u64 range, int slice_log2, RjGeomHost* g);
size_t rj_hist_entries(const RjGeomHost& g);
void launch_rj_partition(hipStream_t s, void* jit_fn, const DevProgram& P, i64 n, const KeySpec& K, const HashTable& T, int payload_via, const RjGeomHost& g,
                         u64* rec, u64* rec_out, int32_t* hist, void* scan_ws, size_t scan_ws_bytes);
int rj_probe_geometry(i64 n, i64* wpw_out);
void launch_rj_probe(hipStream_t s, const u64* rec, const int32_t* n_live, const HashTable& T, int join_type, uint32_t* seg_build, uint32_t* seg_probe,
                     uint32_t* seg_counts, int nblocks, i64 wpw);
void launch_bitmap_select(hipStream_t s, const u64* present, const u64* visited, int matched, i64 nwords, i64 n, u64* bitmap,
                          uint32_t* block_counts, int nblocks, i64 wpb);
void launch_join_probe(hipStream_t s, void* jit_fn, const DevProgram& P, i64 n, const KeySpec& K, const HashTable& T, const uint32_t* next,
                       int join_type, int payload_via, int null_equals_null, uint32_t* out_build, uint32_t* out_probe,
                       u64 out_cap, u64* out_count, uint32_t* visited);
int sort_minmax_blocks(i64 n);
void launch_sort_minmax(hipStream_t s, void* jit_fn, const DevProgram& P, i64 n, const SortSpec& S, u64* out, int nblocks, i64 wstep = 1);
int sort_max_passes();
void launch_sort_pack(hipStream_t s, void* jit_fn, const DevProgram& P, i64 n, const SortSpec& S, const SortPack& K, u64* key_lo, u64* key_hi, uint32_t* ids, u64* hist, int hist_passes);
void launch_part_pid(hipStream_t s, void* jit_fn, const DevProgram& P, i64 n, const KeySpec& K, uint32_t nparts, u64* pid_out, uint32_t* ids);
void launch_part_offsets(hipStream_t s, const u64* pid, i64 n, uint32_t nparts, uint32_t* counts_ws, u64* offsets_out, int shift);
void launch_counts_to_ghist(hipStream_t s, const uint32_t* counts, uint32_t np, u64* ghist);
void launch_gather_u64(hipStream_t s, const u64* src, const uint32_t* idx, i64 n, u64* dst);
int sort_small_max();
int sort_direct_max();
void launch_sort_direct(hipStream_t s, const DevProgram& P, i64 n, const SortSpec& S, uint32_t* perm);
void launch_sort_small(hipStream_t s, const u64* klo, const u64* khi, const uint32_t* ids, i64 n, uint32_t* out);
size_t onesweep_ws_bytes(i64 n);
int onesweep_max_passes();
size_t merge_splits_entries(i64 max_len, int n_pairs);
void launch_merge_pairs(hipStream_t s, const u64* klo, const u64* khi, const uint32_t* ids, const i64* pairs, int n_pairs, i64 max_len, i64* splits,
                        u64* klo_out, u64* khi_out, uint32_t* ids_out);
void launch_radix_ghist(hipStream_t s, const u64* keys, i64 n, int shift0, int npasses, u64* ghist);
void launch_onesweep_pass(hipStream_t s, const u64* keys, const uint32_t* vals, i64 n, int shift, u64* gexcl, void* ws, size_t ws_bytes,
                          u64* keys_out, uint32_t* vals_out, int ids_only );
void launch_agg_emit(hipStream_t s, const AggOut& raw, int n_keys, int n_accs, uint32_t n_groups, const AggSoA& soa, const uint32_t* n_groups_dev = nullptr);
void launch_concat_bitmap(hipStream_t s, u64* dst, i64 dst_bit_offset, const uint8_t* src, i64 src_bit_offset, i64 n_bits);
void launch_unpack_utf8_lengths(hipStream_t s, const ulonglong2* packed, i64 n, int32_t* lens_out, uint32_t* too_long);
constexpr int LIKE_MAX_TOKENS = 256;
constexpr int LIKE_MAX_SEGS = 8;
struct LikePattern {
  int32_t n; int32_t regex_mode; uint16_t tok[LIKE_MAX_TOKENS];
  int32_t n_seg, anchored_start, anchored_end, pad;
  int32_t seg_off[LIKE_MAX_SEGS], seg_len[LIKE_MAX_SEGS];
  unsigned long long seg_first8[LIKE_MAX_SEGS], seg_mask8[LIKE_MAX_SEGS];
};
void launch_like_utf8(hipStream_t s, const uint8_t* data, const int32_t* offsets, const uint8_t* validity, const uint32_t* idx, i64 n, const LikePattern& pat, int negated,
                      u64* bits_out, u64* valid_out);
void launch_mark_rows(hipStream_t s, const uint32_t* rows, i64 n, uint8_t* bitmap);
void launch_utf8_compare(hipStream_t s, const uint8_t* adata, const int32_t* aoffs, const uint8_t* avalid, const uint32_t* aidx, const uint8_t* bdata, const int32_t* boffs,
                         const uint8_t* bvalid, const uint32_t* bidx, int32_t blen, i64 n, int op, u64* bits_out, u64* valid_out);
void launch_sort_decode(hipStream_t s, const u64* recs, int rec_shift, i64 n, const SortPack& K, int desc, int nulls_first, int width, void* out, u64* valid_out);
void launch_cross_pairs(hipStream_t s, i64 n_left, i64 n_right, uint32_t* left_rows, uint32_t* right_rows);
void launch_offsets_rebase(hipStream_t s, const int32_t* src, i64 n, int32_t delta, int32_t* dst);
void launch_take_utf8_lengths(hipStream_t s, const int32_t* offsets, const uint8_t* validity, const uint32_t* idx, i64 n, int32_t* lens, u64* valid_out);
void launch_take_utf8_bytes(hipStream_t s, const uint8_t* data, const int32_t* offsets, const uint32_t* idx, i64 n, const int32_t* out_offsets, uint8_t* out, i64 total_bytes);
void launch_unpack_utf8_bytes(hipStream_t s, const ulonglong2* packed, i64 n, const int32_t* offsets, uint8_t* data_out);
void launch_exclusive_scan_i32(hipStream_t s, int32_t* data, i64 n, void* workspace, size_t ws_bytes);
size_t exclusive_scan_ws_bytes(i64 n);
struct Lz4Block { int64_t src; int64_t slot; int32_t len; int32_t pad; };
constexpr int LZ4_UNIT_BLOCK = 0, LZ4_UNIT_STORED = 1, LZ4_UNIT_FRAME_BLOCKS = 2;
constexpr int LZ4_UNIT_BLOCK_CHECKSUM = 1;
struct Lz4Unit { int64_t src, dst, src_len, dst_len; int32_t mode, flags; };
constexpr int64_t LZ4_BLOCK_BYTES = 65536;
inline int64_t lz4_slot_bytes(int64_t len) { return ((len + len / 255 + 16) + 15) & ~(int64_t)15; }
void launch_lz4_compress(hipStream_t s, const uint8_t* src, uint8_t* slots, const Lz4Block* blocks, int n_blocks, int32_t* csize);
void launch_lz4_layout(hipStream_t s, const Lz4Block* blocks, const int32_t* csize, const int32_t* buf_first_block, int n_buffers, int64_t* buf_off, int64_t* buf_len,
                       int64_t* blk_dst);
void launch_lz4_pack(hipStream_t s, const uint8_t* src, const uint8_t* slots, const Lz4Block* blocks, int n_blocks, const int32_t* csize, const int32_t* blk_buffer,
                     const int32_t* buf_first_block, const int64_t* buf_off, const int64_t* buf_len, const int64_t* blk_dst, uint8_t* body);
void launch_lz4_decode(hipStream_t s, const uint8_t* src, int64_t src_bytes, uint8_t* dst, const Lz4Unit* units, int n_units, uint32_t* status);
struct Utf8Piece { const int32_t* tmp; int64_t n; int32_t* dst; int64_t at, dl, start, used; int32_t first, pad; };
void launch_utf8_piece_starts(hipStream_t s, Utf8Piece* pieces, int n_pieces, uint32_t* gap);
void launch_utf8_piece_offsets(hipStream_t s, const Utf8Piece* pieces, int n_pieces, int64_t max_rows);
void launch_utf8_piece_validate(hipStream_t s, const Utf8Piece* pieces, int n_pieces, int64_t max_rows, uint32_t* status);
void launch_utf8_piece_compact(hipStream_t s, const Utf8Piece* pieces, int n_pieces, int64_t max_bytes, const uint8_t* from, uint8_t* to);
enum UnpackMode : int32_t { UNPACK_STORED = 0, UNPACK_SNAPPY = 1, UNPACK_LZ4_BLOCK = 2, UNPACK_LINKED_STORED = 3, UNPACK_ZSTD = 4 };
constexpr uint32_t UNPACKF_MALFORMED = 1u, UNPACKF_ZSTD_DICTIONARY = 8u;
struct UnpackJob { int64_t src, dst, src_len, dst_len, raw_prefix; int32_t mode, pad; int64_t s_off, c_off, f_off, p_base; };
void launch_unpack_pages(hipStream_t s, const uint8_t* src, uint8_t* dst, const UnpackJob* jobs, int n_jobs, uint32_t* status);
size_t zstd_scratch_bytes(int n_pages);
void launch_zstd_pages(hipStream_t s, const uint8_t* src, uint8_t* dst, const UnpackJob* jobs, const int32_t* which, int n, uint8_t* scratch, uint32_t* status);
struct UnpackScratch { DevBuf jobs, resolve, blkmap, cmap, counts, jump_a, jump_b, olen, mark, scan; };
inline bool unpack_job_is_compressed(const UnpackJob& j) { return j.mode == UNPACK_SNAPPY || j.mode == UNPACK_LZ4_BLOCK; }
void unpack_pages_parallel(hipStream_t s, const uint8_t* src, uint8_t* dst, const UnpackJob* jobs, int n, UnpackScratch& X, uint32_t* status);
constexpr int PJ_BLOCK_BYTES = 4096;
void launch_sn_head(hipStream_t s, const uint8_t* src, uint8_t* dst, const UnpackJob* jobs, int n_jobs, uint8_t* mark, uint32_t* resolve, uint32_t* status);
void launch_sn_next(hipStream_t s, const uint8_t* src, const uint2* cmap, int n_cblocks, const UnpackJob* jobs, uint32_t* jump, uint32_t* olen);
// ... 84 lines not shown
```

### arrow-ballista_amd/csrc/kernels_hash.hip

```cpp
#include "gpuq_kernels.h"

namespace gpuq {

constexpr int HBLOCK = 256;
constexpr int HWAVES = HBLOCK / 64;


__device__ __forceinline__ u64 a_load(const u64* p) { return __hip_atomic_load(p, __ATOMIC_RELAXED, __HIP_MEMORY_SCOPE_AGENT); }
__device__ __forceinline__ void a_store(u64* p, u64 v) { __hip_atomic_store(p, v, __ATOMIC_RELAXED, __HIP_MEMORY_SCOPE_AGENT); }
__device__ __forceinline__ u64 a_cas(u64* p, u64 expected, u64 desired) {
  __hip_atomic_compare_exchange_strong(p, &expected, desired, __ATOMIC_RELAXED, __ATOMIC_RELAXED, __HIP_MEMORY_SCOPE_AGENT);
  return expected;
}
__device__ __forceinline__ u64 a_add(u64* p, u64 v) { return __hip_atomic_fetch_add(p, v, __ATOMIC_RELAXED, __HIP_MEMORY_SCOPE_AGENT); }

__device__ __forceinline__ bool make_key(const KeySpec& K, GPUQ_REGS_CPARAM, u64 (&kw)[MAX_KW], u64& hash) {
  uint32_t knull = 0;
  u64 h = 0x243F6A8885A308D3ull;
#pragma unroll
  for (int k = 0; k < MAX_KEYS; ++k) {
    if (k < K.n_keys) {
      const int r = __builtin_amdgcn_readfirstlane(K.key_reg[k]);
      const bool isn = (rnulls >> r) & 1;
      const u64 lo = isn ? 0 : rlo[r], hi = isn ? 0 : rhi[r];
// ... 348 lines not shown
  const int lane = gpuq::lane();
  RunsLane r;
  r.active_mask = __ballot(active);
  const u64 under = lane ? runs_lanes_le(r.active_mask, lane - 1) : 0ull;
  const u64 near_key = __shfl(key, under ? 63 - __builtin_clzll(under) : 0);
  r.prev_p1 = under ? near_key + 1 : last_p1;
  const bool below = lane ? ((r.active_mask >> (lane - 1)) & 1ull) != 0 : below63;
  r.head = runs_head(active, below, r.prev_p1, key);
  const u64 top_key = __shfl(key, r.active_mask ? 63 - __builtin_clzll(r.active_mask) : 0);
  if (r.active_mask) last_p1 = top_key + 1;
  below63 = (r.active_mask >> 63) != 0;
  return r;
}
template <int MAXC, class Body>
__device__ __forceinline__ u64 runs_walk(const DevProgram& P, const i64 n, const KeySpec& K, const i64 ws, const i64 wps, Body body) {
  bool below63 = false; u64 last_p1 = 0;
  for_rows_in_flight<MAXC>(P, n, ws > 0 ? ws - 1 : 0, 1, [&](const i64 w, const i64, const bool active, GPUQ_REGS_PARAM) {
    const u64 key = active ? pack_state_key(K, GPUQ_REGS) : 0;
    if (w < ws) {
      const int a63 = __shfl((int)active, 63); const u64 k63 = __shfl(key, 63);
      below63 = a63 != 0; last_p1 = a63 ? k63 + 1 : 0;
      return;
    }
    const RunsLane r = runs_word(active, key, below63, last_p1);
    body(key, active, r, GPUQ_REGS);
  }, ws + wps);
  return last_p1;
}

template <int MAXC>
__device__ __forceinline__ void k_agg_runs_count_body(const DevProgram P, const i64 n_arg, const KeySpec K, const RunsGeom G) {
  const i64 n = rows_of(P, n_arg);
  const i64 s = (i64)blockIdx.x * HWAVES + wave();
  if (s >= G.nsegs) return;
  uint32_t heads = 0; u64 first_p1 = 0; bool bad = false;
  const u64 last_p1 = runs_walk<MAXC>(P, n, K, s * G.wps, G.wps, [&](const u64 key, const bool, const RunsLane& r, GPUQ_REGS_CPARAM) {
    heads += (uint32_t)__popcll(__ballot(r.head));
    bad = bad || runs_out_of_order(r.head, r.prev_p1, key);
    const u64 open = __ballot(r.head && r.prev_p1 == 0);
    const u64 open_key = __shfl(key, open ? __builtin_ctzll(open) : 0);
    if (open) first_p1 = open_key + 1;
  });
  if (__ballot(bad) && lane() == 0) atomicOr(P.flags, FLAG_AGG_RUNS);
  if (lane() == 0) { G.counts[s] = heads; G.seg_last[s] = last_p1; G.seg_first[s] = first_p1; }
}
#ifndef GPUQ_JIT
template <int MAXC>
__global__ void __launch_bounds__(HBLOCK) k_agg_runs_count(const DevProgram P, const i64 n, const KeySpec K, const RunsGeom G) { k_agg_runs_count_body<MAXC>(P, n, K, G); }
#elif GPUQ_JIT_KERNEL == GPUQ_SINK_AGG_RUNS_COUNT
extern "C" __global__ void __launch_bounds__(HBLOCK) gpuq_jit_entry(const DevProgram P, const i64 n, const KeySpec K, const RunsGeom G) { k_agg_runs_count_body<0>(P, n, K, G); }
#endif

#ifndef GPUQ_JIT
__global__ void __launch_bounds__(1024) k_agg_runs_order(const RunsGeom G, uint32_t* __restrict__ flags) {
  bool bad = false;
  block_walk_scan<MaxOp>((int)G.nsegs, (u64)0, [&](const int i) { return G.seg_last[i]; },
                         [&](const int i, const u64 before) { const u64 f = G.seg_first[i]; bad = bad || (f != 0 && f <= before); }, (u64*)nullptr);
  if (bad) atomicOr(flags, FLAG_AGG_RUNS);
}
__global__ void __launch_bounds__(HBLOCK) k_fill_cells(ulonglong2* __restrict__ cells, const i64 n, const u64 lo, const u64 hi) {
  for (i64 i = (i64)blockIdx.x * HBLOCK + threadIdx.x; i < n; i += (i64)gridDim.x * HBLOCK) cells[i] = make_ulonglong2(lo, hi);
}
#endif

template <int MAXC>
__device__ __forceinline__ void k_agg_runs_write_body(const DevProgram P, const i64 n_arg, const KeySpec K, const AggSpec A, const RunsGeom G, const AggSoA soa, const uint32_t cap) {
  if (__hip_atomic_load(P.flags, __ATOMIC_RELAXED, __HIP_MEMORY_SCOPE_AGENT) & FLAG_AGG_RUNS) return;
  const i64 n = rows_of(P, n_arg);
  const i64 s = (i64)blockIdx.x * HWAVES + wave();
  if (s >= G.nsegs) return;
  const int lane = gpuq::lane();
  const uint32_t base = G.counts[s];
  uint32_t heads = 0;
  runs_walk<MAXC>(P, n, K, s * G.wps, G.wps, [&](const u64 key, const bool active, const RunsLane& r, GPUQ_REGS_CPARAM) {
    if (r.active_mask == 0) return;
    const u64 head_mask = __ballot(r.head);
    const bool start = r.head | !active | (lane == 0);
    const u64 start_mask = __ballot(start);
    const bool tail = active && (lane == 63 || ((start_mask >> (lane + 1)) & 1ull));
    const uint32_t g = runs_out_row(base, heads, head_mask, lane);
    const bool fits = active && g < cap;
    if (r.head && g >= cap) atomicOr(P.flags, FLAG_GROUP_OVERFLOW);
    if (r.head && fits) emit_state_key(key, K, soa, g);
    const bool interior = runs_piece_interior(head_mask, start_mask, lane);
    for (int a = 0; a < A.n_accs; ++a) {
      const int kind = A.acc_kind[a];
      u64 vlo, vhi;
      bool any = acc_operand(A, a, GPUQ_REGS, vlo, vhi) && active;
      if (!any) { vlo = acc_identity(kind, 0); vhi = acc_identity(kind, 1); }
      acc_wave_segscan(kind, lane, start, vlo, vhi, any);
      if (tail && fits) {
        u64* cell = (u64*)(soa.acc_col[a] + g);
        if (interior) { cell[0] = vlo; cell[1] = vhi; }
        else if (any) acc_fold<__HIP_MEMORY_SCOPE_AGENT>(cell, kind, vlo, vhi);
      }
    }
    heads += (uint32_t)__popcll(head_mask);
  });
}
#ifndef GPUQ_JIT
template <int MAXC>
__global__ void __launch_bounds__(HBLOCK) k_agg_runs_write(const DevProgram P, const i64 n, const KeySpec K, const AggSpec A, const RunsGeom G, const AggSoA soa, const uint32_t cap) {
  k_agg_runs_write_body<MAXC>(P, n, K, A, G, soa, cap);
}
#elif GPUQ_JIT_KERNEL == GPUQ_SINK_AGG_RUNS_WRITE
extern "C" __global__ void __launch_bounds__(HBLOCK) gpuq_jit_entry(const DevProgram P, const i64 n, const KeySpec K, const AggSpec A, const RunsGeom G, const AggSoA soa, const uint32_t cap) {
  k_agg_runs_write_body<0>(P, n, K, A, G, soa, cap);
}
#endif

// ... 913 lines not shown
  const int grid = (int)(need < cap ? (need ? need : 1) : cap);
  hipLaunchKernelGGL(k_ht_init, dim3(grid), dim3(HBLOCK), 0, s, T, A ? *A : dummy, A ? 1 : 0);
}
void launch_agg_hash(hipStream_t s, void* jit_fn, const DevProgram& P, i64 n, const KeySpec& K, const AggSpec& A, const HashTable& T) {
  if (n <= 0) return;
  launch_sink(jit_fn, P.n_cols, GPUQ_PICK(k_agg_hash), dim3(hgrid(n, 8)), dim3(HBLOCK), 0, s, P, n, K, A, T);
}
void launch_key_sample(hipStream_t s, const DevProgram& P, i64 n, const KeySpec& K, i64 stride, i64 nsample, uint32_t* bitmap, u64 nbits, unsigned long long* passed) {
  if (n <= 0 || nsample <= 0) return;
  launch_sink(nullptr, P.n_cols, GPUQ_PICK(k_key_sample), dim3(hgrid(nsample, 8)), dim3(HBLOCK), 0, s, P, n, K, stride, nsample, bitmap, nbits - 1, passed);
}
void launch_agg_origin_pick(hipStream_t s, const DevProgram& pick, i64 n, const OriginPick* origins_dev, unsigned int* first_row) {
  HIPCHECK(hipMemsetAsync(first_row, 0xFF, MAX_ORIGINS * sizeof(unsigned int), s));
  const i64 steps = (n + HBLOCK - 1) / HBLOCK;
  if (steps > 0) launch_sink(nullptr, pick.n_cols, GPUQ_PICK(k_agg_origin_find), dim3((unsigned)std::min<i64>(steps, ORIGIN_FIND_BLOCKS)), dim3(HBLOCK), 0, s, pick, n, origins_dev, first_row);
  launch_sink(nullptr, pick.n_cols, GPUQ_PICK(k_agg_origin_store), dim3(1), dim3(64), 0, s, pick, origins_dev, (const unsigned int*)first_row);
}
uint32_t agg_lds_slots(const HashTable& T) {
  const size_t bytes = (size_t)(T.slot_words + 1) * 8;
  uint32_t cap = 1; while ((size_t)cap * 2 * bytes <= 32768) cap *= 2;
  return cap >= 128 ? cap : 0;
}
int agg_lds_grid(i64 n) { return hgrid(n, 4); }
void launch_agg_lds(hipStream_t s, void* jit_fn, const DevProgram& P, i64 n, const KeySpec& K, const AggSpec& A, const HashTable& T, u64* fstage, int n_fsum) {
  if (n <= 0) return;
  const uint32_t lcap = agg_lds_slots(T);
  const size_t lds = (size_t)lcap * (T.slot_words + 1) * 8;
  const int grid = agg_lds_grid(n);
  launch_sink(jit_fn, P.n_cols, GPUQ_PICK(k_agg_lds), dim3(grid), dim3(HBLOCK), lds, s, P, n, K, A, T, lcap, fstage, n_fsum);
  if (fstage && n_fsum > 0) {
    const u64 items = T.n_slots * (u64)n_fsum;
    const u64 need = (items + HWAVES - 1) / HWAVES, cap = (u64)num_cus() * 8;
    hipLaunchKernelGGL(k_fsum_stage_reduce, dim3((unsigned)(need < cap ? (need ? need : 1) : cap)), dim3(HBLOCK), 0, s, T, A, (const u64*)fstage, n_fsum, (uint32_t)grid);
  }
}
void launch_agg_hash_extract(hipStream_t s, const KeySpec& K, const AggSpec& A, const HashTable& T, const AggOut& out, uint32_t* flags, const AggSoA* soa) {
  AggSoA none{};
  u64 need = (T.n_slots + (u64)HBLOCK * 16 - 1) / ((u64)HBLOCK * 16);
  const u64 cap = (u64)num_cus() * 16;
  const int grid = (int)(need < cap ? (need ? need : 1) : cap);
  hipLaunchKernelGGL(k_agg_hash_extract, dim3(grid), dim3(HBLOCK), 0, s, K, A, T, out, flags, soa ? *soa : none);
}
RunsGeom agg_runs_geometry(i64 n) {
  RunsGeom G{};
  const i64 nwords = (n + 63) >> 6, max_segs = (i64)num_cus() * 8 * HWAVES;
  G.wps = std::max<i64>((nwords + max_segs - 1) / max_segs, 2);
  G.nsegs = (int32_t)((nwords + G.wps - 1) / G.wps);
  return G;
}
void launch_agg_runs_count(hipStream_t s, void* jit_fn, const DevProgram& P, i64 n, const KeySpec& K, const RunsGeom& G) {
  if (G.nsegs <= 0) return;
  launch_sink(jit_fn, P.n_cols, GPUQ_PICK(k_agg_runs_count), dim3((G.nsegs + HWAVES - 1) / HWAVES), dim3(HBLOCK), 0, s, P, n, K, G);
}
void launch_agg_runs_order(hipStream_t s, const RunsGeom& G, uint32_t* flags) {
  if (G.nsegs <= 0) return;
  hipLaunchKernelGGL(k_agg_runs_order, dim3(1), dim3(1024), 0, s, G, flags);
}
void launch_agg_runs_write(hipStream_t s, void* jit_fn, const DevProgram& P, i64 n, const KeySpec& K, const AggSpec& A, const RunsGeom& G, const AggSoA& soa, uint32_t cap) {
  if (G.nsegs <= 0) return;
  launch_sink(jit_fn, P.n_cols, GPUQ_PICK(k_agg_runs_write), dim3((G.nsegs + HWAVES - 1) / HWAVES), dim3(HBLOCK), 0, s, P, n, K, A, G, soa, cap);
}
void launch_fill_cells(hipStream_t s, ulonglong2* cells, i64 n, u64 lo, u64 hi) {
  if (n <= 0) return;
  const i64 need = (n + HBLOCK - 1) / HBLOCK, cap = (i64)num_cus() * 16;
  hipLaunchKernelGGL(k_fill_cells, dim3((unsigned)(need < cap ? need : cap)), dim3(HBLOCK), 0, s, cells, n, lo, hi);
}
void launch_agg_bucket_id(hipStream_t s, void* jit_fn, const DevProgram& P, i64 n, const KeySpec& K, u64 bucket_mask, u64* bid, uint32_t* ids) {
  if (n <= 0) return;
  launch_sink(jit_fn, P.n_cols, GPUQ_PICK(k_agg_bucket_id), dim3(hgrid(n, 8)), dim3(HBLOCK), 0, s, P, n, K, bucket_mask, bid, ids);
}
void launch_bucket_bounds(hipStream_t s, const u64* sorted_bid, i64 n, u64 nbuckets, uint32_t* bounds, int shift) {
  const u64 need = (nbuckets + 1 + HBLOCK - 1) / HBLOCK;
  hipLaunchKernelGGL(k_bucket_bounds, dim3((unsigned)(need < 4096 ? need : 4096)), dim3(HBLOCK), 0, s, sorted_bid, n, nbuckets, bounds, shift);
}
void launch_agg_bucket(hipStream_t s, void* jit_fn, const DevProgram& P, const KeySpec& K, const AggSpec& A, const uint32_t* ids, const uint32_t* bounds, uint32_t nbuckets,
                       uint32_t cap, int slot_words, const AggOut& out) {
  const size_t lds = (size_t)cap * slot_words * 8;
  u64 grid = nbuckets; const u64 gcap = (u64)num_cus() * 8; if (grid > gcap) grid = gcap; if (grid < 1) grid = 1;
  launch_sink(jit_fn, P.n_cols, GPUQ_PICK(k_agg_bucket), dim3((unsigned)grid), dim3(HBLOCK), lds, s, P, K, A, ids, bounds, nbuckets, cap, slot_words, out);
}
bool launch_join_build(hipStream_t s, void* jit_fn, const DevProgram& P, i64 n, const KeySpec& K, const HashTable& T, uint32_t* next, uint32_t* present,
                       int payload_via, int null_equals_null, const SemiProbe* semi) {
  if (n <= 0) return true;
  SemiProbe S{}; if (semi) S = *semi;
  if (semi && !jit_fn && P.n_cols > 8) return false;
  const auto semi_pick = [](auto M) { return &k_join_build<(decltype(M)::value < 8 ? decltype(M)::value : 8), true>; };
  const auto plain_pick = [](auto M) { return &k_join_build<decltype(M)::value, false>; };
  const dim3 grid(hgrid(n, 8)), block(HBLOCK);
  if (semi) launch_sink(jit_fn, P.n_cols, semi_pick, grid, block, 0, s, P, n, K, T, next, present, payload_via, null_equals_null, S);
  else launch_sink(jit_fn, P.n_cols, plain_pick, grid, block, 0, s, P, n, K, T, next, present, payload_via, null_equals_null, S);
  return true;
}

#ifndef GPUQ_JIT
__global__ void __launch_bounds__(HBLOCK) k_bitmap_select(const u64* __restrict__ present, const u64* __restrict__ visited, const int matched,
                                                          const i64 nwords, const i64 n, u64* __restrict__ bitmap,
                                                          uint32_t* __restrict__ block_counts, const i64 wpb) {
  __shared__ uint32_t wc[HWAVES];
  const i64 w0 = (i64)blockIdx.x * wpb;
  i64 w1 = w0 + wpb; if (w1 > nwords) w1 = nwords;
  uint32_t cnt = 0;
  for (i64 w = w0 + threadIdx.x; w < w1; w += HBLOCK) {
    u64 m = present[w] & (matched ? visited[w] : ~visited[w]);
    if (w == nwords - 1 && (n & 63)) m &= (1ull << (n & 63)) - 1;
    bitmap[w] = m; cnt += (uint32_t)__popcll(m);
  }
  const uint32_t t = block_sum<HWAVES>(cnt, wc);
  if (threadIdx.x == 0) block_counts[blockIdx.x] = t;
}
// ... 73 lines not shown
```

### arrow-ballista_amd/csrc/kernels_sort.hip

```cpp
#include "gpuq_kernels.h"

namespace gpuq {

constexpr int SBLOCK = 256;
constexpr int SWAVES = SBLOCK / 64;
constexpr int RADIX = 256;

__device__ __forceinline__ i128 sort_view(u64 lo, u64 hi, int kind) {
  if (kind == 1) { const i64 k = f64_total_key(lo); return (i128)k; }
  if (kind == 2) hi ^= 0x8000000000000000ull;
  return mk128(lo, hi);
}

struct MinMax { u64 mn_lo, mn_hi, mx_lo, mx_hi; uint32_t fl; };
__device__ __forceinline__ void mm_init(MinMax& m) { m.mn_lo = ~0ull; m.mn_hi = 0x7FFFFFFFFFFFFFFFull; m.mx_lo = 0; m.mx_hi = 0x8000000000000000ull; m.fl = 0; }
__device__ __forceinline__ void mm_update(MinMax& m, i128 v) {
  if (v < mk128(m.mn_lo, m.mn_hi)) { m.mn_lo = (u64)v; m.mn_hi = (u64)((u128)v >> 64); }
  if (v > mk128(m.mx_lo, m.mx_hi)) { m.mx_lo = (u64)v; m.mx_hi = (u64)((u128)v >> 64); }
}
__device__ __forceinline__ void mm_row(MinMax& m, const SortSpec& S, int k, GPUQ_REGS_CPARAM) {
  if (k < S.n_keys) {
    const int r = __builtin_amdgcn_readfirstlane(S.reg[k]);
    const bool isn = (rnulls >> r) & 1;
    if (isn) m.fl |= 2u;
    else {
      m.fl |= 1u; mm_update(m, sort_view(rlo[r], rhi[r], S.kind[k]));
      if (S.kind[k] == 2) { const uint32_t len = (uint32_t)(rlo[r] & 0xFF) << 8; if (len > (m.fl & 0xFF00u)) m.fl = (m.fl & ~0xFF00u) | len; }
    }
  }
}
__device__ __forceinline__ void mm_reduce_store(MinMax& m, int k, u64 (*red)[MAX_SORT_KEYS][5]) {
  for (int off = 32; off > 0; off >>= 1) {
    const i128 omn = mk128(__shfl_xor(m.mn_lo, off), __shfl_xor(m.mn_hi, off));
    const i128 omx = mk128(__shfl_xor(m.mx_lo, off), __shfl_xor(m.mx_hi, off));
    if (omn < mk128(m.mn_lo, m.mn_hi)) { m.mn_lo = (u64)omn; m.mn_hi = (u64)((u128)omn >> 64); }
    if (omx > mk128(m.mx_lo, m.mx_hi)) { m.mx_lo = (u64)omx; m.mx_hi = (u64)((u128)omx >> 64); }
    { const uint32_t of = __shfl_xor(m.fl, off); const uint32_t ml = (of & 0xFF00u) > (m.fl & 0xFF00u) ? (of & 0xFF00u) : (m.fl & 0xFF00u); m.fl = ((m.fl | of) & 0xFFu) | ml; }
  }
  if (lane() == 0) { red[wave()][k][0] = m.mn_lo; red[wave()][k][1] = m.mn_hi; red[wave()][k][2] = m.mx_lo; red[wave()][k][3] = m.mx_hi; red[wave()][k][4] = m.fl; }
}
template <int MAXC>
__device__ __forceinline__ void k_sort_minmax_body(const DevProgram P, const i64 n_arg, const SortSpec S, u64* __restrict__ out, const i64 wstep) {
  const i64 n = rows_of(P, n_arg);
  __shared__ u64 red[SWAVES][MAX_SORT_KEYS][5];
  MinMax m0, m1, m2, m3;
  mm_init(m0); mm_init(m1); mm_init(m2); mm_init(m3);
  const i64 nw_all = (n + 63) >> 6;
  const i64 nwords = wstep > 1 ? (nw_all + wstep - 1) / wstep + 1 : nw_all;
  for (i64 w = (i64)blockIdx.x * SWAVES + wave(); w < nwords; w += (i64)gridDim.x * SWAVES) {
    const i64 wi = w * wstep < nw_all ? w * wstep : nw_all - 1;
    const i64 pos = (wi << 6) + lane();
    if (pos >= n) continue;
    GPUQ_REGS_DECL;
// ... 170 lines not shown
    GPUQ_REGS_DECL;
    (void)GPUQ_EVAL(MAXC, P, pos);
    u64 h = 0x243F6A8885A308D3ull;
#pragma unroll
    for (int k = 0; k < MAX_KEYS; ++k) {
      if (k < K.n_keys) {
        const int r = __builtin_amdgcn_readfirstlane(K.key_reg[k]);
        const bool isn = (rnulls >> r) & 1;
        h = hash_combine(h, isn ? 0 : rlo[r], (K.key_wide[k] && !isn) ? rhi[r] : 0, isn);
      }
    }
    if (!ids) { pid_out[pos] = ((u64)(h % nparts) << 32) | (u64)(uint32_t)pos; continue; }
    pid_out[pos] = h % nparts;
    ids[pos] = (uint32_t)pos;
  }
}
#ifndef GPUQ_JIT
template <int MAXC>
__global__ void __launch_bounds__(SBLOCK) k_part_pid(const DevProgram P, const i64 n, const KeySpec K, const uint32_t nparts,
                                                     u64* __restrict__ pid_out, uint32_t* __restrict__ ids) { k_part_pid_body<MAXC>(P, n, K, nparts, pid_out, ids); }
#elif GPUQ_JIT_KERNEL == GPUQ_SINK_PART_PID
extern "C" __global__ void __launch_bounds__(SBLOCK) gpuq_jit_entry(const DevProgram P, const i64 n, const KeySpec K, const uint32_t nparts,
                                                     u64* __restrict__ pid_out, uint32_t* __restrict__ ids) { k_part_pid_body<0>(P, n, K, nparts, pid_out, ids); }
#endif

#ifndef GPUQ_JIT
__global__ void __launch_bounds__(SBLOCK) k_pid_count(const u64* __restrict__ pid, const i64 n, const uint32_t np, uint32_t* __restrict__ counts, const int shift) {
  extern __shared__ uint32_t hist[];
  const bool lds = np <= 8192;
  if (lds) { for (uint32_t d = threadIdx.x; d < np; d += SBLOCK) hist[d] = 0; __syncthreads(); }
  for (i64 i = (i64)blockIdx.x * SBLOCK + threadIdx.x; i < n; i += (i64)gridDim.x * SBLOCK) {
    const uint32_t d = (uint32_t)(pid[i] >> shift);
    if (lds) atomicAdd(&hist[d], 1u); else atomicAdd(&counts[d], 1u);
  }
  if (lds) { __syncthreads(); for (uint32_t d = threadIdx.x; d < np; d += SBLOCK) { const uint32_t c = hist[d]; if (c) atomicAdd(&counts[d], c); } }
}
#endif
#ifndef GPUQ_JIT
__global__ void __launch_bounds__(1024) k_part_scan(const uint32_t* __restrict__ counts, const uint32_t np, u64* __restrict__ offsets) {
  block_walk_scan<SumOp>(np, (u64)0, [&](const uint32_t i) { return (u64)counts[i]; }, [&](const uint32_t i, const u64 before) { offsets[i] = before; }, offsets + np);
}
#endif

#ifndef GPUQ_JIT
__global__ void __launch_bounds__(SBLOCK) k_gather_u64(const u64* __restrict__ src, const uint32_t* __restrict__ idx, const i64 n, u64* __restrict__ dst) {
  for (i64 i = (i64)blockIdx.x * SBLOCK + threadIdx.x; i < n; i += (i64)gridDim.x * SBLOCK) dst[i] = src[idx[i]];
}
#endif

#ifndef GPUQ_JIT
#ifndef GPUQ_JIT
constexpr u64 LB_AGG = 1ull << 62, LB_PREFIX = 2ull << 62, LB_MASK = (1ull << 62) - 1;
constexpr int GHIST_MAX_PASSES = 8;
__global__ void __launch_bounds__(SBLOCK) k_radix_ghist(const u64* __restrict__ keys, const i64 n, const int shift0, const int npasses, u64* __restrict__ ghist) {
  __shared__ uint32_t cnt[GHIST_MAX_PASSES][RADIX];
  for (int i = threadIdx.x; i < GHIST_MAX_PASSES * RADIX; i += SBLOCK) (&cnt[0][0])[i] = 0;
  __syncthreads();
  for (i64 i = (i64)blockIdx.x * SBLOCK + threadIdx.x; i < n; i += (i64)gridDim.x * SBLOCK) {
    const u64 k = keys[i] >> shift0;
    for (int p = 0; p < npasses; ++p) atomicAdd(&cnt[p][(uint32_t)(k >> (8 * p)) & 0xFFu], 1u);
  }
  __syncthreads();
  for (int i = threadIdx.x; i < npasses * RADIX; i += SBLOCK) { const uint32_t c = (&cnt[0][0])[i]; if (c) atomicAdd((unsigned long long*)&ghist[i], (unsigned long long)c); }
}
__global__ void __launch_bounds__(RADIX) k_radix_ghist_scan(u64* __restrict__ ghist) {
  __shared__ u64 ws[RADIX / 64];
  u64* h = ghist + (size_t)blockIdx.x * RADIX;
  h[threadIdx.x] = block_excl_scan<RADIX / 64>(h[threadIdx.x], ws);
}
template <bool HASVAL, int OROUNDS>
__global__ void __launch_bounds__(SBLOCK) k_onesweep(const u64* __restrict__ keys, const uint32_t* __restrict__ vals, const i64 n, const int shift,
                                                     const u64* __restrict__ gexcl, u64* __restrict__ look, uint32_t* __restrict__ ticket,
                                                     u64* __restrict__ keys_out, uint32_t* __restrict__ vals_out, const int ids_only) {
  __shared__ u64 sk[(SBLOCK * OROUNDS)];
  __shared__ uint32_t sv[HASVAL ? (SBLOCK * OROUNDS) : 1];
  __shared__ uint32_t wcnt[SWAVES][RADIX];
  __shared__ uint32_t dstart[RADIX];
  __shared__ u64 gbase[RADIX];
  __shared__ uint32_t wsum[SWAVES];
  __shared__ uint32_t s_tile;
  const int t = threadIdx.x, w = wave(), l = lane();
  const u64 lt = (1ull << l) - 1;
  if (t == 0) s_tile = atomicAdd(ticket, 1u);
  for (int i = t; i < SWAVES * RADIX; i += SBLOCK) (&wcnt[0][0])[i] = 0;
  __syncthreads();
  const i64 T = (i64)s_tile;
  const i64 s0 = T * (SBLOCK * OROUNDS);
  if (s0 >= n) return;
  const i64 b = s0 + (SBLOCK * OROUNDS) < n ? s0 + (SBLOCK * OROUNDS) : n;
  const i64 w0 = s0 + (i64)w * ((SBLOCK * OROUNDS) / SWAVES);
  u64 k[OROUNDS]; uint32_t v[HASVAL ? OROUNDS : 1]; uint32_t pos[OROUNDS];
#pragma unroll
  for (int r = 0; r < OROUNDS; ++r) {
    const i64 i = w0 + r * 64 + l;
    const bool act = i < b;
    k[r] = act ? keys[i] : 0;
    if (HASVAL) v[r] = act ? vals[i] : 0;
  }
#pragma unroll
  for (int r = 0; r < OROUNDS; ++r) {
    const i64 i = w0 + r * 64 + l;
    const bool act = i < b;
    const uint32_t d = (uint32_t)(k[r] >> shift) & 0xFFu;
    uint32_t dlo = 0, dhi = 0;
#pragma unroll
    for (int bit = 0; bit < 8; bit += 2) {
      const uint32_t s0 = (uint32_t)__builtin_amdgcn_sbfe((int)d, bit, 1), s1 = (uint32_t)__builtin_amdgcn_sbfe((int)d, bit + 1, 1);
      const u64 m0 = __ballot(s0 != 0), m1 = __ballot(s1 != 0);
      dlo = __builtin_amdgcn_bitop3_b32(dlo, (uint32_t)m0, s0, 0xF6); dhi = __builtin_amdgcn_bitop3_b32(dhi, (uint32_t)(m0 >> 32), s0, 0xF6);
      dlo = __builtin_amdgcn_bitop3_b32(dlo, (uint32_t)m1, s1, 0xF6); dhi = __builtin_amdgcn_bitop3_b32(dhi, (uint32_t)(m1 >> 32), s1, 0xF6);
    }
    const u64 same = ~(((u64)dhi << 32) | (u64)dlo) & __ballot(act);
    const uint32_t before = act ? wcnt[w][d] : 0;
    pos[r] = before + (uint32_t)__popcll(same & lt);
    __builtin_amdgcn_wave_barrier();
    if (act && (same >> l) <= 1ull) wcnt[w][d] = before + (uint32_t)__popcll(same);
    __builtin_amdgcn_wave_barrier();
  }
  __syncthreads();
  uint32_t tot = 0;
  {
    uint32_t c[SWAVES];
#pragma unroll
    for (int q = 0; q < SWAVES; ++q) { c[q] = wcnt[q][t]; tot += c[q]; }
    __hip_atomic_store(&look[(size_t)T * RADIX + t], (T == 0 ? LB_PREFIX : LB_AGG) | (u64)tot, __ATOMIC_RELAXED, __HIP_MEMORY_SCOPE_AGENT);
    const uint32_t ds = block_excl_scan<SWAVES>(tot, wsum);
    dstart[t] = ds;
    uint32_t run = ds;
#pragma unroll
    for (int q = 0; q < SWAVES; ++q) { wcnt[q][t] = run; run += c[q]; }
  }
  __syncthreads();
#pragma unroll
  for (int r = 0; r < OROUNDS; ++r) {
    const i64 i = w0 + r * 64 + l;
    if (i < b) { const uint32_t d = (uint32_t)(k[r] >> shift) & 0xFFu; const uint32_t j = wcnt[w][d] + pos[r]; sk[j] = k[r]; if (HASVAL) sv[j] = v[r]; }
  }
  {
    u64 excl = 0;
// ... 66 lines not shown
  __shared__ u64 slo[MTILE]; __shared__ u64 shi[WIDE ? MTILE : 1]; __shared__ uint32_t sid[MTILE];
  const i64 a0 = pairs[3 * blockIdx.y], a1 = pairs[3 * blockIdx.y + 1], a2 = pairs[3 * blockIdx.y + 2];
  const i64 na = a1 - a0, nb = a2 - a1;
  const i64 d0 = (i64)blockIdx.x * MTILE;
  if (d0 >= na + nb) return;
  const i64 d1 = d0 + MTILE < na + nb ? d0 + MTILE : na + nb;
  auto gA = [&](i64 i) -> MKey { return MKey{WIDE ? khi[a0 + i] : 0, klo[a0 + i]}; };
  auto gB = [&](i64 i) -> MKey { return MKey{WIDE ? khi[a1 + i] : 0, klo[a1 + i]}; };
  const i64* sp = splits + (size_t)blockIdx.y * (size_t)(tiles_per_pair + 1) + blockIdx.x;
  const i64 i0 = sp[0], i1 = sp[1];
  const i64 j0 = d0 - i0, j1 = d1 - i1;
  const int ca = (int)(i1 - i0), cb = (int)(j1 - j0);
  for (int q = threadIdx.x; q < ca + cb; q += SBLOCK) {
    const i64 src = q < ca ? a0 + i0 + q : a1 + j0 + (q - ca);
    slo[q] = klo[src]; if (WIDE) shi[q] = khi[src]; sid[q] = ids[src];
  }
  __syncthreads();
  auto lA = [&](int i) -> MKey { return MKey{WIDE ? shi[i] : 0, slo[i]}; };
  auto lB = [&](int i) -> MKey { return MKey{WIDE ? shi[ca + i] : 0, slo[ca + i]}; };
  const int t0 = threadIdx.x * MVT;
  const int total = ca + cb;
  u64 olo[MVT], ohi[MVT]; uint32_t oid[MVT];
  if (t0 < total) {
    int i = merge_path(t0, ca, cb, lA, lB), j = t0 - i;
#pragma unroll
    for (int q = 0; q < MVT; ++q) {
      if (t0 + q >= total) break;
      const bool takeA = j >= cb || (i < ca && mk_le(lA(i), lB(j)));
      const int src = takeA ? i : ca + j;
      olo[q] = slo[src]; ohi[q] = WIDE ? shi[src] : 0; oid[q] = sid[src];
      if (takeA) ++i; else ++j;
    }
  }
  __syncthreads();
  if (t0 < total) {
#pragma unroll
    for (int q = 0; q < MVT; ++q) if (t0 + q < total) { slo[t0 + q] = olo[q]; if (WIDE) shi[t0 + q] = ohi[q]; sid[t0 + q] = oid[q]; }
  }
  __syncthreads();
  for (int q = threadIdx.x; q < total; q += SBLOCK) {
    const i64 dst = a0 + d0 + q;
    klo_out[dst] = slo[q]; if (WIDE) khi_out[dst] = shi[q]; ids_out[dst] = sid[q];
  }
}
#endif

static int sgrid(i64 n, int blocks_per_cu) { return grid_for_words(n, SWAVES, blocks_per_cu); }
int sort_minmax_blocks(i64 n) { return sgrid(n, 4); }
void launch_sort_minmax(hipStream_t s, void* jit_fn, const DevProgram& P, i64 n, const SortSpec& S, u64* out, int nblocks, i64 wstep) {
  if (wstep < 1) wstep = 1;
  launch_sink(jit_fn, P.n_cols, GPUQ_PICK(k_sort_minmax), dim3(nblocks), dim3(SBLOCK), 0, s, P, n, S, out, wstep);
}
int sort_max_passes() { return SORT_MAX_PASSES; }
void launch_sort_pack(hipStream_t s, void* jit_fn, const DevProgram& P, i64 n, const SortSpec& S, const SortPack& K, u64* key_lo, u64* key_hi, uint32_t* ids, u64* hist, int hist_passes) {
  if (n <= 0) return;
  if (hist) (void)hipMemsetAsync(hist, 0, (size_t)hist_passes * RADIX * 8, s);
  if (hist && K.check == 1) (void)hipMemsetAsync(hist + (size_t)SORT_MAX_PASSES * RADIX, 0, 8, s);
  launch_sink(jit_fn, P.n_cols, GPUQ_PICK(k_sort_pack), dim3(sgrid(n, 8)), dim3(SBLOCK), 0, s, P, n, S, K, key_lo, key_hi, ids, hist, hist_passes);
}
void launch_part_pid(hipStream_t s, void* jit_fn, const DevProgram& P, i64 n, const KeySpec& K, uint32_t nparts, u64* pid_out, uint32_t* ids) {
  if (n <= 0) return;
  launch_sink(jit_fn, P.n_cols, GPUQ_PICK(k_part_pid), dim3(sgrid(n, 8)), dim3(SBLOCK), 0, s, P, n, K, nparts, pid_out, ids);
}
__global__ void __launch_bounds__(RADIX) k_counts_to_ghist(const uint32_t* __restrict__ counts, const uint32_t np, u64* __restrict__ ghist) {
  ghist[threadIdx.x] = threadIdx.x < np ? (u64)counts[threadIdx.x] : 0;
}
void launch_counts_to_ghist(hipStream_t s, const uint32_t* counts, uint32_t np, u64* ghist) {
  hipLaunchKernelGGL(k_counts_to_ghist, dim3(1), dim3(RADIX), 0, s, counts, np, ghist);
}
void launch_part_offsets(hipStream_t s, const u64* pid, i64 n, uint32_t nparts, uint32_t* counts_ws, u64* offsets_out, int shift) {
  (void)hipMemsetAsync(counts_ws, 0, (size_t)(nparts + 1) * 4, s);
  i64 need = (n + SBLOCK - 1) / SBLOCK; const i64 cap = (i64)num_cus() * 8; if (need < 1) need = 1;
  hipLaunchKernelGGL(k_pid_count, dim3((int)(need < cap ? need : cap)), dim3(SBLOCK), nparts <= 8192 ? (size_t)nparts * 4 : 0, s, pid, n, nparts, counts_ws, shift);
  hipLaunchKernelGGL(k_part_scan, dim3(1), dim3(1024), 0, s, (const uint32_t*)counts_ws, nparts, offsets_out);
}
void launch_gather_u64(hipStream_t s, const u64* src, const uint32_t* idx, i64 n, u64* dst) {
  if (n <= 0) return;
  i64 need = (n + SBLOCK - 1) / SBLOCK; const i64 cap = (i64)num_cus() * 16;
  hipLaunchKernelGGL(k_gather_u64, dim3((int)(need < cap ? need : cap)), dim3(SBLOCK), 0, s, src, idx, n, dst);
}
constexpr int SMALL_SORT_MAX = 2048;
__global__ void __launch_bounds__(1024) k_sort_small(const u64* __restrict__ klo, const u64* __restrict__ khi, const uint32_t* __restrict__ ids,
                                                     const int n, uint32_t* __restrict__ out) {
  __shared__ u64 slo[SMALL_SORT_MAX], shi[SMALL_SORT_MAX];
  __shared__ uint32_t sid[SMALL_SORT_MAX];
  int m = 2; while (m < n) m <<= 1;
  for (int i = threadIdx.x; i < m; i += 1024) {
    if (i < n) { slo[i] = klo[i]; shi[i] = khi ? khi[i] : 0ull; sid[i] = ids[i]; }
    else { slo[i] = ~0ull; shi[i] = ~0ull; sid[i] = 0xFFFFFFFFu; }
  }
  __syncthreads();
  for (int k = 2; k <= m; k <<= 1) {
    for (int j = k >> 1; j > 0; j >>= 1) {
      for (int i = threadIdx.x; i < m; i += 1024) {
        const int x = i ^ j;
        if (x > i) {
          const u64 ah = shi[i], al = slo[i], bh = shi[x], bl = slo[x];
          const uint32_t ai = sid[i], bi = sid[x];
          const bool a_gt_b = ah != bh ? ah > bh : (al != bl ? al > bl : ai > bi);
          const bool up = (i & k) == 0;
          if (a_gt_b == up) { shi[i] = bh; slo[i] = bl; sid[i] = bi; shi[x] = ah; slo[x] = al; sid[x] = ai; }
        }
      }
      __syncthreads();
    }
  }
  for (int i = threadIdx.x; i < n; i += 1024) out[i] = sid[i];
}
int sort_small_max() { return SMALL_SORT_MAX; }
int sort_direct_max() { return SORT_DIRECT_MAX; }
void launch_sort_direct(hipStream_t s, const DevProgram& P, i64 n, const SortSpec& S, uint32_t* perm) {
  if (n <= 0) return;
  launch_sink(nullptr, P.n_cols, GPUQ_PICK(k_sort_direct), dim3(1), dim3(SORT_DIRECT_MAX), 0, s, P, (int)n, S, perm);
}
void launch_sort_small(hipStream_t s, const u64* klo, const u64* khi, const uint32_t* ids, i64 n, uint32_t* out) {
  if (n > 0) hipLaunchKernelGGL(k_sort_small, dim3(1), dim3(1024), 0, s, klo, khi, ids, (int)n, out);
}

constexpr int OS_ROUNDS_PACKED = 32, OS_ROUNDS_KV = 24;
size_t onesweep_ws_bytes(i64 n) { const i64 tiles = (n + SBLOCK * OS_ROUNDS_KV - 1) / (SBLOCK * OS_ROUNDS_KV); return (size_t)tiles * RADIX * 8 + 256; }
int onesweep_max_passes() { return GHIST_MAX_PASSES; }
void launch_radix_ghist(hipStream_t s, const u64* keys, i64 n, int shift0, int npasses, u64* ghist) {
  if (n <= 0 || npasses <= 0) return;
  (void)hipMemsetAsync(ghist, 0, (size_t)npasses * RADIX * 8, s);
  i64 need = (n + SBLOCK * 16 - 1) / (SBLOCK * 16); const i64 cap = (i64)num_cus() * 8;
  hipLaunchKernelGGL(k_radix_ghist, dim3((unsigned)std::max<i64>(1, std::min(need, cap))), dim3(SBLOCK), 0, s, keys, n, shift0, npasses, ghist);
}
__global__ void __launch_bounds__(SBLOCK) k_sort_decode(const u64* __restrict__ recs, const int rec_shift, const i64 n, const SortPack K, const int desc, const int nulls_first,
                                                        const int width, uint8_t* __restrict__ out, u64* __restrict__ valid_out) {
  const i64 nwords = (n + 63) >> 6;
  const i128 base = mk128(K.base_lo[0], K.base_hi[0]);
  const u64 vmask = K.vbits[0] >= 64 ? ~0ull : ((1ull << K.vbits[0]) - 1);
  for (i64 w = (i64)blockIdx.x * SWAVES + wave(); w < nwords; w += (i64)gridDim.x * SWAVES) {
    const i64 i = (w << 6) + lane();
    bool valid = false;
    if (i < n) {
      const u64 comp = recs[i] >> rec_shift;
      bool isn = false;
      if (K.null_bit[0] >= 0) isn = (((comp >> K.null_bit[0]) & 1ull) != 0) != (nulls_first != 0);
      const u64 field = comp & vmask;
      const i128 v = isn ? (i128)0 : (desc ? base - (i128)field : base + (i128)field);
      valid = !isn;
      switch (width) {
        case 1: out[i] = (uint8_t)v; break;
        case 2: ((uint16_t*)out)[i] = (uint16_t)v; break;
        case 4: ((uint32_t*)out)[i] = (uint32_t)v; break;
        case 8: ((u64*)out)[i] = (u64)v; break;
        default: ((ulonglong2*)out)[i] = make_ulonglong2((u64)v, (u64)((u128)v >> 64)); break;
      }
    }
    if (valid_out) { const u64 vb = __ballot(valid); if (lane() == 0) valid_out[w] = vb; }
  }
}
void launch_sort_decode(hipStream_t s, const u64* recs, int rec_shift, i64 n, const SortPack& K, int desc, int nulls_first, int width, void* out, u64* valid_out) {
  if (n <= 0) return;
  i64 need = ((n + 63) / 64 + SWAVES - 1) / SWAVES; const i64 cap = (i64)num_cus() * 16;
  hipLaunchKernelGGL(k_sort_decode, dim3((unsigned)(need < cap ? need : cap)), dim3(SBLOCK), 0, s, recs, rec_shift, n, K, desc, nulls_first, width, (uint8_t*)out, valid_out);
}

void launch_onesweep_pass(hipStream_t s, const u64* keys, const uint32_t* vals, i64 n, int shift, u64* gexcl, void* ws, size_t ws_bytes,
                          u64* keys_out, uint32_t* vals_out, int ids_only) {
  if (n <= 0) return;
  const int rounds = vals ? OS_ROUNDS_KV : OS_ROUNDS_PACKED;
  const i64 tile = (i64)SBLOCK * rounds;
  const i64 tiles = (n + tile - 1) / tile;
  (void)hipMemsetAsync(ws, 0, ws_bytes, s);
  u64* look = (u64*)ws; uint32_t* ticket = (uint32_t*)((char*)ws + (size_t)tiles * RADIX * 8);
  hipLaunchKernelGGL(k_radix_ghist_scan, dim3(1), dim3(RADIX), 0, s, gexcl);
  if (vals) hipLaunchKernelGGL((k_onesweep<true, OS_ROUNDS_KV>), dim3((unsigned)tiles), dim3(SBLOCK), 0, s, keys, vals, n, shift, (const u64*)gexcl, look, ticket, keys_out, vals_out, ids_only);
  else hipLaunchKernelGGL((k_onesweep<false, OS_ROUNDS_PACKED>), dim3((unsigned)tiles), dim3(SBLOCK), 0, s, keys, vals, n, shift, (const u64*)gexcl, look, ticket, keys_out, vals_out, ids_only);
}

size_t merge_splits_entries(i64 max_len, int n_pairs) { return (size_t)n_pairs * (size_t)((max_len + MTILE - 1) / MTILE + 1); }
void launch_merge_pairs(hipStream_t s, const u64* klo, const u64* khi, const uint32_t* ids, const i64* pairs, int n_pairs, i64 max_len, i64* splits,
                        u64* klo_out, u64* khi_out, uint32_t* ids_out) {
  if (n_pairs <= 0 || max_len <= 0) return;
  const int tpp = (int)((max_len + MTILE - 1) / MTILE);
  const dim3 pg((unsigned)((tpp + 1 + SBLOCK - 1) / SBLOCK), (unsigned)n_pairs), mg((unsigned)tpp, (unsigned)n_pairs);
  if (khi) {
    hipLaunchKernelGGL(k_merge_partition<true>, pg, dim3(SBLOCK), 0, s, klo, khi, pairs, tpp, splits);
    hipLaunchKernelGGL(k_merge_pairs<true>, mg, dim3(SBLOCK), 0, s, klo, khi, ids, pairs, (const i64*)splits, tpp, klo_out, khi_out, ids_out);
  } else {
    hipLaunchKernelGGL(k_merge_partition<false>, pg, dim3(SBLOCK), 0, s, klo, khi, pairs, tpp, splits);
    hipLaunchKernelGGL(k_merge_pairs<false>, mg, dim3(SBLOCK), 0, s, klo, khi, ids, pairs, (const i64*)splits, tpp, klo_out, khi_out, ids_out);
  }
}

#endif

}
```

Measured before the change: 176.2 billion rows/s.

## Prune agg count program, fuse runs scan/order, double-buffer onesweep look-back

Builds a pruned expression program for the aggregate runs-count sink that evaluates only the key columns and predicate, so dead accumulator columns are neither loaded nor computed. It merges the block-count scan and the runs-order check into one kernel. Radix sort passes now double-buffer the look-back workspace, with each pass zeroing the next pass's buffer, so there is one memset per sort instead of per pass. The global-histogram scans are batched into one multi-block launch, and the sort-pack grid is capped by rows per block. These changes add complexity and new invariants around workspace sizing and ticket alternation.

```diff
diff --git a/arrow-ballista_amd/csrc/agg_compile.cpp b/arrow-ballista_amd/csrc/agg_compile.cpp
--- a/arrow-ballista_amd/csrc/agg_compile.cpp
+++ b/arrow-ballista_amd/csrc/agg_compile.cpp
@@ -471,6 +471,7 @@
   for (auto& k : keys.nodes) key_slots.push_back(ec.add_output(k));
   for (size_t i = 0; i < accs.size(); ++i) if (accs[i].arg) acc_slots[i] = ec.add_output(accs[i].arg);
   R.prog = ec.finish();
+  R.heads = ec.prune(R.prog, (int)keys.nodes.size());
   if (!s.origin_of.empty()) {
     if (d.has("predicate")) s.pick.add_predicate(ec.from_json(d.at("predicate")));
     R.pick = s.pick.finish();
diff --git a/arrow-ballista_amd/csrc/agg_compile.h b/arrow-ballista_amd/csrc/agg_compile.h
--- a/arrow-ballista_amd/csrc/agg_compile.h
+++ b/arrow-ballista_amd/csrc/agg_compile.h
@@ -14,6 +14,7 @@
   std::string mode = "Single", strategy = "auto";
   i64 expected_groups = 0;
   CompiledProgram prog;
+  CompiledProgram heads;
   CompiledProgram pick; int n_origins = 0;
   AggSpec agg{}; KeySpec keys{};
   std::vector<DType> key_types, acc_types;
diff --git a/arrow-ballista_amd/csrc/capi.cpp b/arrow-ballista_amd/csrc/capi.cpp
--- a/arrow-ballista_amd/csrc/capi.cpp
+++ b/arrow-ballista_amd/csrc/capi.cpp
@@ -60,6 +60,7 @@
   struct PostChunk { CompiledProgram prog; DevBuf code; int first_out = 0; };
   std::deque<PostChunk> posts; Schema post_schema;
   CompiledProgram pick; DevBuf pick_code, origins_dev, origin_rows; int n_origins = 0;
+  CompiledProgram heads; DevBuf heads_code;
   i64 expected_groups = 0;
   int agg_path = 0;
   int join_type = JT_INNER; int null_eq = 0; bool build_side_rows = true;
@@ -144,6 +145,12 @@
 }
 
 DevProgram bind_input(gpuq_op* op, const gpuq_input* in) { return bind_program(op->prog, op->in_schema, op->code_dev.as<DevCode>(), op->flags_dev.as<uint32_t>(), in); }
+DevProgram heads_program(const gpuq_op* op, const DevProgram& P) {
+  DevProgram H = P;
+  H.code = op->heads_code.as<DevCode>(); H.n_insns = op->heads.n_insns;
+  for (size_t c = 0; c < op->heads.col_dead.size(); ++c) if (op->heads.col_dead[c]) { H.cols[c] = DevCol{}; H.cols[c].cls = CC_NONE; }
+  return H;
+}
 void check_payload_via(int payload_via, const gpuq_input* in) { if (payload_via < 0 || payload_via > in->n_via) throw std::runtime_error("payload_via out of range"); }
 void check_row_limit(i64 n, const char* what) { if (n >= (1ll << 31)) throw Unsupported(std::string(what) + " of >= 2^31 rows in one call"); }
 void need_exact_rows(const gpuq_input* in, const char* what) {
@@ -278,11 +285,9 @@
 }
 
 u64* bucket_records(hipStream_t s, u64* rec, u64* rec2, i64 n, int npass, const PassBufs& pass, uint32_t* ids_out, int last_mode) {
-  for (int p = 0; p < npass; ++p) {
-    const bool last = p + 1 == npass;
-    launch_onesweep_pass(s, rec, nullptr, n, 32 + 8 * p, pass.hist.as<u64>() + (size_t)p * 256, pass.look.p, pass.look_bytes, rec2, last ? ids_out : nullptr, last ? last_mode : 0);
-    std::swap(rec, rec2);
-  }
+  launch_radix_ghist_scan(s, pass.hist.as<u64>(), npass);
+  uint32_t* none = nullptr; uint32_t* none2 = nullptr;
+  launch_onesweep_passes(s, rec, none, rec2, none2, n, 32, npass, pass.hist.as<u64>(), pass.look.p, pass.look_bytes, ids_out, last_mode);
   return rec;
 }
 
@@ -346,6 +351,7 @@
       AggCompiled c = compile_aggregate(op->in_schema, d);
       op->mode = c.mode; op->strategy = c.strategy; op->expected_groups = c.expected_groups; op->refuse = c.refuse;
       op->prog = std::move(c.prog); upload_code(op->prog, op->code_dev);
+      op->heads = std::move(c.heads); if (op->heads.pruned()) upload_code(op->heads, op->heads_code);
       op->agg = c.agg; op->keys = c.keys;
       op->key_types = std::move(c.key_types); op->acc_types = std::move(c.acc_types); op->acc_bits = std::move(c.acc_bits);
       op->post_schema = std::move(c.post_schema); op->out_fields = std::move(c.out_fields);
@@ -513,6 +519,7 @@
     compile_op(op, d);
     g_upload = true;
     std::string eval = op->prog.jit_src;
+    if (kernel_id == GPUQ_SINK_AGG_RUNS_COUNT && op->kind == K_AGG && op->heads.pruned()) eval = op->heads.jit_src;
     if (kernel_id == GPUQ_SINK_AGG_TINY && op->kind == K_AGG) eval += agg_tiny_spec(op, (int)d.get_i64("jit_gmax", 4));
     const std::string src = jit_full_source(eval, kernel_id);
     if (src.size() + 1 > cap) throw Capacity("source needs " + std::to_string(src.size() + 1) + " bytes");
@@ -741,9 +748,10 @@
       raw.n_groups = n_groups_dev(op);
       if (reset) reset_flags(op, s);
       if (G.nsegs <= 0) { HIPCHECK(hipMemsetAsync(raw.n_groups, 0, 8, s)); return; }
-      { SinkJit jit(op, op->prog, GPUQ_SINK_AGG_RUNS_COUNT, n); launch_agg_runs_count(s, jit.fn, P, n, Krun, G); }
-      launch_scan_block_counts(s, G.counts, G.nsegs, (u64*)raw.n_groups);
-      launch_agg_runs_order(s, G, op->flags_dev.as<uint32_t>());
+      const bool pruned = op->heads.pruned();
+      const DevProgram Pc = pruned ? heads_program(op, P) : P;
+      { SinkJit jit(op, pruned ? op->heads : op->prog, GPUQ_SINK_AGG_RUNS_COUNT, n); launch_agg_runs_count(s, jit.fn, Pc, n, Krun, G); }
+      launch_agg_runs_scan_order(s, G, (u64*)raw.n_groups, op->flags_dev.as<uint32_t>());
     };
     auto launch_runs_write = [&](const i64 rcap) {
       raw.cap = (int32_t)rcap;
@@ -1345,14 +1353,11 @@
       return;
     }
     void* lws = W.pass.lookback(n); const size_t lwb = W.pass.look_bytes;
+    launch_radix_ghist_scan(s, ghist, np_all);
     auto run_passes = [&](int bits, int shift0, int pass0, bool last_word) {
       const int np = (bits + 7) / 8;
       if (np == 0) { if (last_word) HIPCHECK(hipMemcpyAsync(perm_out, ids, (size_t)n * 4, hipMemcpyDeviceToDevice, s)); return; }
-      for (int p = 0; p < np; ++p) {
-        const bool final_pass = last_word && p + 1 == np;
-        launch_onesweep_pass(s, klo, ids, n, shift0 + 8 * p, ghist + (size_t)(pass0 + p) * 256, lws, lwb, klo2, final_pass ? perm_out : ids2, final_pass ? (decode ? (packed ? 2 : 0) : 1) : 0);
-        std::swap(klo, klo2); if (!final_pass) std::swap(ids, ids2);
-      }
+      launch_onesweep_passes(s, klo, ids, klo2, ids2, n, shift0, np, ghist + (size_t)pass0 * 256, lws, lwb, last_word ? perm_out : nullptr, decode ? (packed ? 2 : 0) : 1);
     };
     if (packed) {
       run_passes(total, 32, 0, true);
diff --git a/arrow-ballista_amd/csrc/expr_compile.cpp b/arrow-ballista_amd/csrc/expr_compile.cpp
--- a/arrow-ballista_amd/csrc/expr_compile.cpp
+++ b/arrow-ballista_amd/csrc/expr_compile.cpp
@@ -752,13 +752,16 @@
   };
   std::map<Node*, int> remaining = uses;
   auto release = [&](Node* c0) { Node* c = rep(c0); if (--remaining[c] == 0) busy[reg[c]] = false; };
+  fin_insns_.clear();
   for (Node* n : order) {
     if (n->kind == Node::COL) continue;
+    const int first_insn = C.n_insns;
     if (n->kind == Node::LIT) {
       const int d = alloc(); reg[n] = d;
-      if (n->param >= 0) { const int slot = imm_new(0, 0, true); param_slot_[n] = slot; C.param_imm.push_back({n->param, slot}); emit(OP_IMM, d, 0, 0, (uint32_t)slot); continue; }
+      if (n->param >= 0) { const int slot = imm_new(0, 0, true); param_slot_[n] = slot; C.param_imm.push_back({n->param, slot}); emit(OP_IMM, d, 0, 0, (uint32_t)slot); fin_insns_[n] = {first_insn, 1}; continue; }
       if (n->lit_null) { emit(OP_IMM, d, 0, 0, (uint32_t)imm_index(0, 0)); emit(OP_NULLIF0, d, d, d, 0); }
       else emit(OP_IMM, d, 0, 0, (uint32_t)imm_index(n->lit_lo, n->lit_hi));
+      fin_insns_[n] = {first_insn, C.n_insns - first_insn};
       continue;
     }
     const int a = n->ch.size() > 0 ? reg.at(rep(n->ch[0].get())) : 0;
@@ -768,7 +771,9 @@
     for (auto& c : n->ch) release(c.get());
     const int d = alloc(); reg[n] = d;
     emit(n->op, d, a, b, imm);
-  }
+    fin_insns_[n] = {first_insn, 1};
+  }
+  fin_order_ = order; fin_reg_ = reg;
   for (size_t i = 0; i < imms.size(); ++i) { C.code.imm_lo[i] = imms[i].first; C.code.imm_hi[i] = imms[i].second; }
   C.pred_reg = pred_ ? reg.at(rep(pred_.get())) : -1;
   for (auto& o : outs_) {
@@ -777,6 +782,42 @@
   for (Node* n : order) if (n->kind == Node::OPN && (n->op == OP_ADDC || n->op == OP_SUBC || n->op == OP_MULC)) C.checks_overflow = true;
   C.jit_src = jit_source(C, order, reg);
   return C;
+}
+
+CompiledProgram ExprCompiler::prune(const CompiledProgram& C, int n_outs) {
+  auto rep = [](Node* n) { while (n->kind == Node::OPN && n->op == OP_MOV) n = n->ch[0].get(); return n; };
+  if (n_outs < 0 || n_outs > (int)outs_.size() || C.out_reg.size() != outs_.size()) throw std::runtime_error("prune: not the program finish() returned");
+  std::set<Node*> live;
+  std::function<void(Node*)> mark = [&](Node* n0) {
+    Node* n = rep(n0);
+    if (!live.insert(n).second) return;
+    for (auto& c : n->ch) mark(c.get());
+  };
+  if (pred_) mark(pred_.get());
+  for (int k = 0; k < n_outs; ++k) mark(outs_[(size_t)k].get());
+  std::vector<Node*> order;
+  for (Node* n : fin_order_) if (live.count(n)) order.push_back(n);
+  if (order.size() == fin_order_.size()) return CompiledProgram();
+  for (Node* n : order) if (n->kind == Node::LIT && n->param >= 0) return CompiledProgram();
+  CompiledProgram R;
+  R.code = C.code; R.n_insns = 0;
+  for (Node* n : order) {
+    auto it = fin_insns_.find(n);
+    if (it == fin_insns_.end()) continue;
+    for (int i = 0; i < it->second.second; ++i) R.code.insns[R.n_insns++] = C.code.insns[it->second.first + i];
+  }
+  for (int i = R.n_insns; i < MAX_INSNS; ++i) R.code.insns[i] = DevInsn{};
+  R.col_field = C.col_field; R.col_loose = C.col_loose;
+  R.col_dead.assign(C.col_field.size(), true);
+  for (Node* n : order) if (n->kind == Node::COL) for (size_t c = 0; c < C.col_field.size(); ++c) if (C.col_field[c] == n->col) R.col_dead[c] = false;
+  R.pred_reg = C.pred_reg;
+  for (int k = 0; k < n_outs; ++k) {
+    R.out_reg.push_back(C.out_reg[(size_t)k]); R.out_type.push_back(C.out_type[(size_t)k]); R.out_nullable.push_back(C.out_nullable[(size_t)k]);
+    R.out_key.push_back(C.out_key[(size_t)k]); R.out_bits.push_back(C.out_bits[(size_t)k]);
+  }
+  for (Node* n : order) if (n->kind == Node::OPN && (n->op == OP_ADDC || n->op == OP_SUBC || n->op == OP_MULC)) R.checks_overflow = true;
+  R.jit_src = jit_source(R, order, fin_reg_);
+  return R;
 }
 
 std::string ExprCompiler::jit_source(const CompiledProgram& C, const std::vector<Node*>& order, const std::map<Node*, int>& ) {
@@ -800,8 +841,9 @@
     if (ty == "ulonglong2") touch += "  asm volatile(\"\" :: \"v\"(w." + nm + ".x), \"v\"(w." + nm + ".y));\n";
     else if (ty != "bool") touch += "  asm volatile(\"\" :: \"v\"(w." + nm + "));\n";
   };
+  auto dead = [&](size_t c) { return c < C.col_dead.size() && C.col_dead[c]; };
   bool via_used[MAX_VIA + 1] = {false, false, false, false};
-  for (size_t c = 0; c < C.col_field.size(); ++c) via_used[schema_.fields[C.col_field[c]].side] = true;
+  for (size_t c = 0; c < C.col_field.size(); ++c) if (!dead(c)) via_used[schema_.fields[C.col_field[c]].side] = true;
   LP("const uint32_t row0 = (uint32_t)pos; (void)row0;");
   LL("const uint32_t row0 = (uint32_t)pos; (void)row0;");
   L("const uint32_t row0 = (uint32_t)pos; (void)row0;");
@@ -821,6 +863,7 @@
     narrow128[c] = seen && all_narrow;
   }
   for (size_t c = 0; c < C.col_field.size(); ++c) {
+    if (dead(c)) continue;
     const Field& f = schema_.fields[C.col_field[c]];
     const std::string cs = std::to_string(c), row = "row" + std::to_string(f.side);
     LL("const DevCol& col" + cs + " = P.cols[" + cs + "];");
@@ -869,7 +912,7 @@
   }
   for (size_t c = 0; c < C.col_field.size(); ++c) {
     const Field& f = schema_.fields[C.col_field[c]];
-    if (f.raw128 || f.type.id != T_UTF8) continue;
+    if (dead(c) || f.raw128 || f.type.id != T_UTF8) continue;
     const std::string cs = std::to_string(c);
     L("const int32_t len" + cs + " = o" + cs + "b - o" + cs + "a;");
     L("const uint8_t* sp" + cs + " = (const uint8_t*)col" + cs + ".data + o" + cs + "a;");
@@ -1066,7 +1109,7 @@
   emit_pred();
   L("uint32_t nm = 0;");
   std::set<int> done;
-  for (size_t k = 0; k < outs_.size(); ++k) {
+  for (size_t k = 0; k < C.out_reg.size(); ++k) {
     Node* o = rep(outs_[k].get());
     const int r = C.out_reg[k];
     if (done.count(r)) continue;
diff --git a/arrow-ballista_amd/csrc/expr_compile.h b/arrow-ballista_amd/csrc/expr_compile.h
--- a/arrow-ballista_amd/csrc/expr_compile.h
+++ b/arrow-ballista_amd/csrc/expr_compile.h
@@ -71,6 +71,8 @@
   int n_insns = 0;
   std::vector<int> col_field;
   std::vector<bool> col_loose;
+  std::vector<bool> col_dead;
+  bool pruned() const { return !col_dead.empty(); }
   int pred_reg = -1;
   std::vector<int> out_reg;
   std::vector<DType> out_type;
@@ -109,6 +111,7 @@
   void add_predicate(NodeP e);
   int add_output(NodeP e);
   CompiledProgram finish();
+  CompiledProgram prune(const CompiledProgram& C, int n_outs);
   const Schema& schema() const { return schema_; }
 
  private:
@@ -117,6 +120,9 @@
   std::vector<NodeP> outs_;
   std::map<std::string, NodeP> interned_;
   std::map<const Node*, int> param_slot_;
+  std::vector<Node*> fin_order_;
+  std::map<Node*, int> fin_reg_;
+  std::map<Node*, std::pair<int, int>> fin_insns_;
   NodeP intern(NodeP n);
   std::string jit_source(const CompiledProgram& C, const std::vector<Node*>& order, const std::map<Node*, int>& reg);
 };
diff --git a/arrow-ballista_amd/csrc/gpuq_dev.h b/arrow-ballista_amd/csrc/gpuq_dev.h
--- a/arrow-ballista_amd/csrc/gpuq_dev.h
+++ b/arrow-ballista_amd/csrc/gpuq_dev.h
@@ -35,6 +35,7 @@
   CC_I8 = 7, CC_I16 = 8, CC_U8 = 9, CC_U16 = 10,
   CC_F32 = 11,
   CC_STRQ = 6,
+  CC_NONE = 15,
 };
 
 struct DevCol {
diff --git a/arrow-ballista_amd/csrc/gpuq_kernels.h b/arrow-ballista_amd/csrc/gpuq_kernels.h
--- a/arrow-ballista_amd/csrc/gpuq_kernels.h
+++ b/arrow-ballista_amd/csrc/gpuq_kernels.h
@@ -307,7 +307,7 @@
 void launch_agg_hash_extract(hipStream_t s, const KeySpec& K, const AggSpec& A, const HashTable& T, const AggOut& out, uint32_t* flags, const AggSoA* soa = nullptr);
 RunsGeom agg_runs_geometry(i64 n);
 void launch_agg_runs_count(hipStream_t s, void* jit_fn, const DevProgram& P, i64 n, const KeySpec& K, const RunsGeom& G);
-void launch_agg_runs_order(hipStream_t s, const RunsGeom& G, uint32_t* flags);
+void launch_agg_runs_scan_order(hipStream_t s, const RunsGeom& G, u64* n_groups_out, uint32_t* flags);
 void launch_agg_runs_write(hipStream_t s, void* jit_fn, const DevProgram& P, i64 n, const KeySpec& K, const AggSpec& A, const RunsGeom& G, const AggSoA& soa, uint32_t cap);
 void launch_fill_cells(hipStream_t s, ulonglong2* cells, i64 n, u64 lo, u64 hi);
 bool launch_join_build(hipStream_t s, void* jit_fn, const DevProgram& P, i64 n, const KeySpec& K, const HashTable& T, uint32_t* next, uint32_t* present,
@@ -349,8 +349,9 @@
 void launch_merge_pairs(hipStream_t s, const u64* klo, const u64* khi, const uint32_t* ids, const i64* pairs, int n_pairs, i64 max_len, i64* splits,
                         u64* klo_out, u64* khi_out, uint32_t* ids_out);
 void launch_radix_ghist(hipStream_t s, const u64* keys, i64 n, int shift0, int npasses, u64* ghist);
-void launch_onesweep_pass(hipStream_t s, const u64* keys, const uint32_t* vals, i64 n, int shift, u64* gexcl, void* ws, size_t ws_bytes,
-                          u64* keys_out, uint32_t* vals_out, int ids_only );
+void launch_radix_ghist_scan(hipStream_t s, u64* ghist, int npasses);
+void launch_onesweep_passes(hipStream_t s, u64*& keys, uint32_t*& vals, u64*& keys2, uint32_t*& vals2, i64 n, int shift0, int np, const u64* gexcl,
+                            void* ws, size_t ws_bytes, uint32_t* final_vals_out, int final_mode );
 void launch_agg_emit(hipStream_t s, const AggOut& raw, int n_keys, int n_accs, uint32_t n_groups, const AggSoA& soa, const uint32_t* n_groups_dev = nullptr);
 void launch_concat_bitmap(hipStream_t s, u64* dst, i64 dst_bit_offset, const uint8_t* src, i64 src_bit_offset, i64 n_bits);
 void launch_unpack_utf8_lengths(hipStream_t s, const ulonglong2* packed, i64 n, int32_t* lens_out, uint32_t* too_long);
diff --git a/arrow-ballista_amd/csrc/kernels_hash.hip b/arrow-ballista_amd/csrc/kernels_hash.hip
--- a/arrow-ballista_amd/csrc/kernels_hash.hip
+++ b/arrow-ballista_amd/csrc/kernels_hash.hip
@@ -424,10 +424,40 @@
 #endif
 
 #ifndef GPUQ_JIT
-__global__ void __launch_bounds__(1024) k_agg_runs_order(const RunsGeom G, uint32_t* __restrict__ flags) {
+__global__ void __launch_bounds__(1024) k_agg_runs_scan_order(const RunsGeom G, u64* __restrict__ n_groups_out, uint32_t* __restrict__ flags) {
+  __shared__ u64 wsum[16], wmax[16];
+  const int n = (int)G.nsegs, w = wave(), l = lane();
+  const int per = (((n + 15) / 16) + 63) & ~63;
+  const int a = w * per, b = a + per < n ? a + per : n;
+  u64 sum = 0, mx = 0;
+  for (int i = a + l; i < b; i += 64) { sum += (u64)G.counts[i]; mx = MaxOp()(mx, G.seg_last[i]); }
+  sum = wave_reduce<SumOp>(sum); mx = wave_reduce<MaxOp>(mx);
+  if (l == 0) { wsum[w] = sum; wmax[w] = mx; }
+  __syncthreads();
+  if (threadIdx.x == 0) {
+    u64 rs = 0, rm = 0;
+    for (int k = 0; k < 16; ++k) { const u64 vs = wsum[k], vm = wmax[k]; wsum[k] = rs; wmax[k] = rm; rs += vs; rm = MaxOp()(rm, vm); }
+    *n_groups_out = rs;
+  }
+  __syncthreads();
+  u64 csum = wsum[w], cmax = wmax[w];
   bool bad = false;
-  block_walk_scan<MaxOp>((int)G.nsegs, (u64)0, [&](const int i) { return G.seg_last[i]; },
-                         [&](const int i, const u64 before) { const u64 f = G.seg_first[i]; bad = bad || (f != 0 && f <= before); }, (u64*)nullptr);
+  u64 c = 0, last = 0, first = 0;
+  if (a + l < b) { c = (u64)G.counts[a + l]; last = G.seg_last[a + l]; first = G.seg_first[a + l]; }
+  for (int i0 = a; i0 < b; i0 += 64) {
+    const int i = i0 + l, nx = i + 64;
+    u64 c2 = 0, last2 = 0, first2 = 0;
+    if (nx < b) { c2 = (u64)G.counts[nx]; last2 = G.seg_last[nx]; first2 = G.seg_first[nx]; }
+    const u64 xs = wave_incl_scan<SumOp>(c), xm = wave_incl_scan<MaxOp>(last);
+    u64 bs = __shfl_up(xs, 1), bm = __shfl_up(xm, 1);
+    if (l == 0) { bs = 0; bm = 0; }
+    if (i < b) {
+      G.counts[i] = (uint32_t)(csum + bs);
+      bad = bad || (first != 0 && first <= MaxOp()(cmax, bm));
+    }
+    csum += __shfl(xs, 63); cmax = MaxOp()(cmax, __shfl(xm, 63));
+    c = c2; last = last2; first = first2;
+  }
   if (bad) atomicOr(flags, FLAG_AGG_RUNS);
 }
 __global__ void __launch_bounds__(HBLOCK) k_fill_cells(ulonglong2* __restrict__ cells, const i64 n, const u64 lo, const u64 hi) {
@@ -1447,9 +1477,9 @@
   if (G.nsegs <= 0) return;
   launch_sink(jit_fn, P.n_cols, GPUQ_PICK(k_agg_runs_count), dim3((G.nsegs + HWAVES - 1) / HWAVES), dim3(HBLOCK), 0, s, P, n, K, G);
 }
-void launch_agg_runs_order(hipStream_t s, const RunsGeom& G, uint32_t* flags) {
+void launch_agg_runs_scan_order(hipStream_t s, const RunsGeom& G, u64* n_groups_out, uint32_t* flags) {
   if (G.nsegs <= 0) return;
-  hipLaunchKernelGGL(k_agg_runs_order, dim3(1), dim3(1024), 0, s, G, flags);
+  hipLaunchKernelGGL(k_agg_runs_scan_order, dim3(1), dim3(1024), 0, s, G, n_groups_out, flags);
 }
 void launch_agg_runs_write(hipStream_t s, void* jit_fn, const DevProgram& P, i64 n, const KeySpec& K, const AggSpec& A, const RunsGeom& G, const AggSoA& soa, uint32_t cap) {
   if (G.nsegs <= 0) return;
diff --git a/arrow-ballista_amd/csrc/kernels_sort.hip b/arrow-ballista_amd/csrc/kernels_sort.hip
--- a/arrow-ballista_amd/csrc/kernels_sort.hip
+++ b/arrow-ballista_amd/csrc/kernels_sort.hip
@@ -1,4 +1,7 @@
 #include "gpuq_kernels.h"
+#ifndef GPUQ_JIT
+#include <cstdlib>
+#endif
 
 namespace gpuq {
 
@@ -275,6 +278,7 @@
 #ifndef GPUQ_JIT
 constexpr u64 LB_AGG = 1ull << 62, LB_PREFIX = 2ull << 62, LB_MASK = (1ull << 62) - 1;
 constexpr int GHIST_MAX_PASSES = 8;
+constexpr int LB_TICKET_STRIDE = 32;
 __global__ void __launch_bounds__(SBLOCK) k_radix_ghist(const u64* __restrict__ keys, const i64 n, const int shift0, const int npasses, u64* __restrict__ ghist) {
   __shared__ uint32_t cnt[GHIST_MAX_PASSES][RADIX];
   for (int i = threadIdx.x; i < GHIST_MAX_PASSES * RADIX; i += SBLOCK) (&cnt[0][0])[i] = 0;
@@ -293,8 +297,14 @@
 }
 template <bool HASVAL, int OROUNDS>
 __global__ void __launch_bounds__(SBLOCK) k_onesweep(const u64* __restrict__ keys, const uint32_t* __restrict__ vals, const i64 n, const int shift,
-                                                     const u64* __restrict__ gexcl, u64* __restrict__ look, uint32_t* __restrict__ ticket,
+                                                     const u64* __restrict__ gexcl, u64* __restrict__ looks, uint32_t* __restrict__ ticket,
                                                      u64* __restrict__ keys_out, uint32_t* __restrict__ vals_out, const int ids_only) {
+  const size_t lwords = (size_t)gridDim.x * RADIX;
+  uint32_t* const tickets = (uint32_t*)(looks + 2 * lwords);
+  const int mine = ticket == tickets ? 0 : 1;
+  u64* const look = looks + (size_t)mine * lwords;
+  u64* const look_next = looks + (size_t)(1 - mine) * lwords;
+  uint32_t* const ticket_next = tickets + (1 - mine) * LB_TICKET_STRIDE;
   __shared__ u64 sk[(SBLOCK * OROUNDS)];
   __shared__ uint32_t sv[HASVAL ? (SBLOCK * OROUNDS) : 1];
   __shared__ uint32_t wcnt[SWAVES][RADIX];
@@ -308,6 +318,8 @@
   for (int i = t; i < SWAVES * RADIX; i += SBLOCK) (&wcnt[0][0])[i] = 0;
   __syncthreads();
   const i64 T = (i64)s_tile;
+  look_next[(size_t)T * RADIX + t] = 0;
+  if (T == 0 && t == 0) *ticket_next = 0;
   const i64 s0 = T * (SBLOCK * OROUNDS);
   if (s0 >= n) return;
   const i64 b = s0 + (SBLOCK * OROUNDS) < n ? s0 + (SBLOCK * OROUNDS) : n;
@@ -480,11 +492,17 @@
   launch_sink(jit_fn, P.n_cols, GPUQ_PICK(k_sort_minmax), dim3(nblocks), dim3(SBLOCK), 0, s, P, n, S, out, wstep);
 }
 int sort_max_passes() { return SORT_MAX_PASSES; }
+constexpr i64 SORT_PACK_ROWS = 2048;
+static i64 sort_pack_rows() {
+  static const i64 r = []() { const char* e = getenv("GPUQ_SORT_PACK_ROWS"); const i64 v = e ? atoll(e) : 0; return v >= 64 ? v : SORT_PACK_ROWS; }();
+  return r;
+}
 void launch_sort_pack(hipStream_t s, void* jit_fn, const DevProgram& P, i64 n, const SortSpec& S, const SortPack& K, u64* key_lo, u64* key_hi, uint32_t* ids, u64* hist, int hist_passes) {
   if (n <= 0) return;
-  if (hist) (void)hipMemsetAsync(hist, 0, (size_t)hist_passes * RADIX * 8, s);
-  if (hist && K.check == 1) (void)hipMemsetAsync(hist + (size_t)SORT_MAX_PASSES * RADIX, 0, 8, s);
-  launch_sink(jit_fn, P.n_cols, GPUQ_PICK(k_sort_pack), dim3(sgrid(n, 8)), dim3(SBLOCK), 0, s, P, n, S, K, key_lo, key_hi, ids, hist, hist_passes);
+  if (hist) (void)hipMemsetAsync(hist, 0, K.check == 1 ? ((size_t)SORT_MAX_PASSES * RADIX + 1) * 8 : (size_t)hist_passes * RADIX * 8, s);
+  int grid = sgrid(n, 8);
+  if (hist) { const i64 by_rows = (n + sort_pack_rows() - 1) / sort_pack_rows(); if (by_rows < grid) grid = (int)by_rows; }
+  launch_sink(jit_fn, P.n_cols, GPUQ_PICK(k_sort_pack), dim3(grid), dim3(SBLOCK), 0, s, P, n, S, K, key_lo, key_hi, ids, hist, hist_passes);
 }
 void launch_part_pid(hipStream_t s, void* jit_fn, const DevProgram& P, i64 n, const KeySpec& K, uint32_t nparts, u64* pid_out, uint32_t* ids) {
   if (n <= 0) return;
@@ -546,7 +564,8 @@
 }
 
 constexpr int OS_ROUNDS_PACKED = 32, OS_ROUNDS_KV = 24;
-size_t onesweep_ws_bytes(i64 n) { const i64 tiles = (n + SBLOCK * OS_ROUNDS_KV - 1) / (SBLOCK * OS_ROUNDS_KV); return (size_t)tiles * RADIX * 8 + 256; }
+static size_t onesweep_used_bytes(i64 tiles) { return 2 * (size_t)tiles * RADIX * 8 + 2 * LB_TICKET_STRIDE * 4; }
+size_t onesweep_ws_bytes(i64 n) { const i64 tiles = (n + SBLOCK * OS_ROUNDS_KV - 1) / (SBLOCK * OS_ROUNDS_KV); return onesweep_used_bytes(tiles); }
 int onesweep_max_passes() { return GHIST_MAX_PASSES; }
 void launch_radix_ghist(hipStream_t s, const u64* keys, i64 n, int shift0, int npasses, u64* ghist) {
   if (n <= 0 || npasses <= 0) return;
@@ -586,17 +605,30 @@
   hipLaunchKernelGGL(k_sort_decode, dim3((unsigned)(need < cap ? need : cap)), dim3(SBLOCK), 0, s, recs, rec_shift, n, K, desc, nulls_first, width, (uint8_t*)out, valid_out);
 }
 
-void launch_onesweep_pass(hipStream_t s, const u64* keys, const uint32_t* vals, i64 n, int shift, u64* gexcl, void* ws, size_t ws_bytes,
-                          u64* keys_out, uint32_t* vals_out, int ids_only) {
-  if (n <= 0) return;
+void launch_radix_ghist_scan(hipStream_t s, u64* ghist, int npasses) {
+  if (npasses > 0) hipLaunchKernelGGL(k_radix_ghist_scan, dim3((unsigned)npasses), dim3(RADIX), 0, s, ghist);
+}
+void launch_onesweep_passes(hipStream_t s, u64*& keys, uint32_t*& vals, u64*& keys2, uint32_t*& vals2, i64 n, int shift0, int np, const u64* gexcl,
+                            void* ws, size_t ws_bytes, uint32_t* final_vals_out, int final_mode) {
+  if (n <= 0 || np <= 0) return;
   const int rounds = vals ? OS_ROUNDS_KV : OS_ROUNDS_PACKED;
   const i64 tile = (i64)SBLOCK * rounds;
   const i64 tiles = (n + tile - 1) / tile;
-  (void)hipMemsetAsync(ws, 0, ws_bytes, s);
-  u64* look = (u64*)ws; uint32_t* ticket = (uint32_t*)((char*)ws + (size_t)tiles * RADIX * 8);
-  hipLaunchKernelGGL(k_radix_ghist_scan, dim3(1), dim3(RADIX), 0, s, gexcl);
-  if (vals) hipLaunchKernelGGL((k_onesweep<true, OS_ROUNDS_KV>), dim3((unsigned)tiles), dim3(SBLOCK), 0, s, keys, vals, n, shift, (const u64*)gexcl, look, ticket, keys_out, vals_out, ids_only);
-  else hipLaunchKernelGGL((k_onesweep<false, OS_ROUNDS_PACKED>), dim3((unsigned)tiles), dim3(SBLOCK), 0, s, keys, vals, n, shift, (const u64*)gexcl, look, ticket, keys_out, vals_out, ids_only);
+  const size_t used = onesweep_used_bytes(tiles);
+  if (used > ws_bytes) throw std::runtime_error("radix passes: look-back workspace too small");
+  (void)hipMemsetAsync(ws, 0, used, s);
+  u64* looks = (u64*)ws; uint32_t* tickets = (uint32_t*)(looks + 2 * (size_t)tiles * RADIX);
+  for (int p = 0; p < np; ++p) {
+    uint32_t* ticket = tickets + (p & 1) * LB_TICKET_STRIDE;
+    const bool final_pass = final_vals_out && p + 1 == np;
+    uint32_t* vout = final_pass ? final_vals_out : vals2;
+    const int mode = final_pass ? final_mode : 0;
+    const u64* base = gexcl + (size_t)p * RADIX;
+    const int shift = shift0 + 8 * p;
+    if (vals) hipLaunchKernelGGL((k_onesweep<true, OS_ROUNDS_KV>), dim3((unsigned)tiles), dim3(SBLOCK), 0, s, (const u64*)keys, (const uint32_t*)vals, n, shift, base, looks, ticket, keys2, vout, mode);
+    else hipLaunchKernelGGL((k_onesweep<false, OS_ROUNDS_PACKED>), dim3((unsigned)tiles), dim3(SBLOCK), 0, s, (const u64*)keys, (const uint32_t*)vals, n, shift, base, looks, ticket, keys2, vout, mode);
+    std::swap(keys, keys2); if (!final_pass) std::swap(vals, vals2);
+  }
 }
 
 size_t merge_splits_entries(i64 max_len, int n_pairs) { return (size_t)n_pairs * (size_t)((max_len + MTILE - 1) / MTILE + 1); }
```

New measurement: 181.7 billion rows/s, median of 6. 1.03x the previous value.
